# MarioCalvarro/circom_cvm

Measured on AMD Instinct MI355X. Metric: constraints simplified/sec (--O2) on 10M-constraint circuit; bit-exact .r1cs, higher is better.
Workload: dtype u64x4 (F_p, 256-bit Montgomery)

## Files before the change

circom_cvm_amd/abi.py:

```python
from __future__ import annotations

import ctypes as C

import numpy as np
import os

PKG = os.path.dirname(os.path.abspath(__file__))
LIB_PATH = os.environ.get("RS_LIB") or os.path.join(PKG, "librs_simplify.so")

U64_MAX = (1 << 64) - 1
PRIME_IDS = {"bn128": 0, "bls12381": 1, "goldilocks": 2, "grumpkin": 3, "pallas": 4,
             "vesta": 5, "secq256r1": 6, "bls12377": 7}
RS_PRIME_CUSTOM = 255
ERRORS = {0: "RS_OK", -1: "RS_E_INVALID", -2: "RS_E_OOM_DEVICE", -3: "RS_E_HIP",
          -4: "RS_E_RCCL", -5: "RS_E_INTERNAL", -6: "RS_E_NODEVICE"}


class RsLc(C.Structure):
    _fields_ = [("n_rows", C.c_uint64), ("nnz", C.c_uint64), ("ptr", C.POINTER(C.c_uint64)),
                ("col", C.POINTER(C.c_uint32)), ("val", C.POINTER(C.c_uint64))]


class RsInput(C.Structure):
    _fields_ = [("prime_id", C.c_uint32), ("prime", C.c_uint64 * 4), ("max_signal", C.c_uint64),
# ... 48 lines not shown
    if n == 0:
        return np.zeros(1, np.uint64), np.zeros(0, np.uint32), np.zeros(0, np.uint64)
    ext = int(lc.nnz)
    col = np.ctypeslib.as_array(lc.col, shape=(max(ext, 1),))
    val = np.ctypeslib.as_array(lc.val, shape=(max(ext, 1) * 4,))
    if layout is None:
        beg = np.ctypeslib.as_array(lc.ptr, shape=(n + 1,)).copy()
        nnz = int(beg[n])
        return beg, col[:nnz].copy(), val[:4 * nnz].copy()
    lp, jp, nj = layout
    lens = np.ctypeslib.as_array(lp, shape=(n,))
    jumps = np.ctypeslib.as_array(jp, shape=(nj,)) if nj else np.zeros(0, np.uint64)
    b = row_starts(lens, jumps)
    ln = (lens & ~np.uint32(ROW_JUMP)).astype(np.int64)
    if n and int((b + ln).max()) > ext:
        raise ValueError("row layout reaches past the block's entries")
    ptr = np.zeros(n + 1, np.uint64)
    np.cumsum(ln, out=ptr[1:])
    idx = np.repeat(b - ptr[:-1].astype(np.int64), ln) + np.arange(int(ptr[n]), dtype=np.int64)
    v4 = val[: 4 * ext].reshape(-1, 4)
    return ptr, col[idx].copy(), v4[idx].reshape(-1).copy()


class RsStats(C.Structure):
    _fields_ = [("total_ms", C.c_double), ("eq_ms", C.c_double), ("cluster_ms", C.c_double),
                ("elim_ms", C.c_double), ("subst_ms", C.c_double), ("final_ms", C.c_double),
                ("apply_kernel_ms", C.c_double), ("apply_kernel_launches", C.c_uint64),
                ("apply_bytes", C.c_uint64), ("elim_kernel_ms", C.c_double),
                ("elim_kernel_launches", C.c_uint64), ("elim_bytes", C.c_uint64),
                ("elim_big_ms", C.c_double), ("elim_small_ms", C.c_double), ("nl_ms", C.c_double),
                ("map_ms", C.c_double), ("rounds_ms", C.c_double),
                ("big_prep_ms", C.c_double), ("big_main_ms", C.c_double), ("big_finish_ms", C.c_double),
                ("big_main_bytes", C.c_uint64), ("big_finish_bytes", C.c_uint64), ("big_launches", C.c_uint64),
                ("rounds", C.c_uint64), ("n_clusters", C.c_uint64),
                ("n_substitutions", C.c_uint64), ("max_cluster", C.c_uint64),
                ("exchange_ms", C.c_double), ("exchange_bytes", C.c_uint64), ("world", C.c_uint64),
                ("head_main_ms", C.c_double), ("head_main_bytes", C.c_uint64), ("head_launches", C.c_uint64),
                ("tail_main_ms", C.c_double), ("tail_main_bytes", C.c_uint64), ("tail_launches", C.c_uint64),
                ("round_fill_ms", C.c_double), ("round_fill_bytes", C.c_uint64),
                ("round_fill_launches", C.c_uint64), ("alg_bytes", C.c_uint64), ("h2d_wait_ms", C.c_double),
                ("d2h_ms", C.c_double), ("host_total_ms", C.c_double), ("write_ms", C.c_double),
                ("tail_fin_ms", C.c_double), ("tail_fin_bytes", C.c_uint64), ("tail_fin_launches", C.c_uint64), ("head_fin_ms", C.c_double), ("head_fin_bytes", C.c_uint64), ("head_fin_launches", C.c_uint64), ("small_ms", C.c_double), ("small_bytes", C.c_uint64), ("small_launches", C.c_uint64), ("prep_ms", C.c_double), ("prep_launches", C.c_uint64), ("cluster_dev_ms", C.c_double), ("cluster_bytes", C.c_uint64), ("cluster_launches", C.c_uint64), ("giant_ms", C.c_double), ("giant_bytes", C.c_uint64), ("giant_launches", C.c_uint64), ("giant_merges", C.c_uint64),
                ("check_ms", C.c_double), ("check_bytes", C.c_uint64), ("check_launches", C.c_uint64),
                ("ragged_ms", C.c_double), ("ragged_bytes", C.c_uint64), ("ragged_launches", C.c_uint64),
                ("gather_ms", C.c_double), ("gather_bytes", C.c_uint64), ("gather_launches", C.c_uint64),
                ("cluster_host_ms", C.c_double),
                ("read_ms", C.c_double), ("read_upload_ms", C.c_double), ("read_kernel_ms", C.c_double),
                ("read_d2h_ms", C.c_double),
                ("sym_write_ms", C.c_double), ("sym_in_ms", C.c_double), ("sym_kernel_ms", C.c_double),
                ("sym_out_ms", C.c_double)]

    def as_dict(self):
        return {k: getattr(self, k) for k, _ in self._fields_}


class RsJsonStats(C.Structure):
    _fields_ = [("write_ms", C.c_double), ("in_ms", C.c_double), ("kernel_ms", C.c_double),
                ("out_ms", C.c_double), ("bytes", C.c_uint64)]

    def as_dict(self):
        return {k: getattr(self, k) for k, _ in self._fields_}


class RsWitness(C.Structure):
    _fields_ = [("prime_id", C.c_uint32), ("prime", C.c_uint64 * 4), ("n8", C.c_uint32), ("n", C.c_uint64),
                ("val", C.POINTER(C.c_uint64))]


WIT_INPUT, WIT_OUTPUT, WIT_LOG = 1, 2, 4
WIT_CLASSES = ("cons_eq", "eq", "linear", "nonlinear", "output", "log")


class RsWitnessReport(C.Structure):
    _fields_ = [("checked", C.c_uint64 * 6), ("failed", C.c_uint64 * 6), ("first_failed", C.c_uint64 * 6),
                ("in_ms", C.c_double), ("kernel_ms", C.c_double), ("total_ms", C.c_double)]

    def as_dict(self):
        d = {k: getattr(self, k) for k in ("in_ms", "kernel_ms", "total_ms")}
        for i, nm in enumerate(WIT_CLASSES):
            first = int(self.first_failed[i])
            d[nm] = {"checked": int(self.checked[i]), "failed": int(self.failed[i]),
                     "first_failed": None if first == U64_MAX else first}
        return d


class RsLiftReport(C.Structure):
    _fields_ = [("n_labels", C.c_uint64), ("n_wires", C.c_uint64), ("lifted", C.c_uint64), ("free_labels", C.c_uint64),
                ("shadowed", C.c_uint64), ("levels", C.c_uint64), ("entries", C.c_uint64),
                ("in_ms", C.c_double), ("kernel_ms", C.c_double), ("total_ms", C.c_double)]

    def as_dict(self):
        return {k: getattr(self, k) for k, _ in self._fields_}

    def counts(self):
        return tuple(int(getattr(self, k)) for k, t in self._fields_ if t is C.c_uint64)


class RsDag(C.Structure):
    _fields_ = [("prime_id", C.c_uint32), ("prime", C.c_uint64 * 4),
                ("n_pub_out", C.c_uint64), ("n_pub_in", C.c_uint64), ("n_priv_in", C.c_uint64),
                ("n_forbidden", C.c_uint64), ("forbidden", C.POINTER(C.c_uint32)),
                ("n_nodes", C.c_uint32), ("main_node", C.c_uint32),
                ("cons_off", C.POINTER(C.c_uint64)), ("a", RsLc), ("b", RsLc), ("c", RsLc),
                ("local_off", C.POINTER(C.c_uint64)), ("locals", C.POINTER(C.c_uint32)),
                ("custom_gate", C.POINTER(C.c_uint8)),
                ("edge_off", C.POINTER(C.c_uint64)), ("edge_to", C.POINTER(C.c_uint32)),
                ("edge_in", C.POINTER(C.c_uint64))]


SYMBOLS = [
    ("rs_last_error", C.c_char_p, []),
    ("rs_abi_version", C.c_int, []),
    ("rs_simplify", C.c_int, [C.POINTER(RsInput), C.POINTER(RsFlags), C.POINTER(C.POINTER(RsOutput))]),
    ("rs_output_free", None, [C.POINTER(RsOutput)]),
    ("rs_engine_create", C.c_int, [C.c_int, C.POINTER(C.c_void_p)]),
    ("rs_engine_load", C.c_int, [C.c_void_p, C.POINTER(RsInput)]),
    ("rs_engine_run", C.c_int, [C.c_void_p, C.POINTER(RsFlags)]),
    ("rs_engine_fetch", C.c_int, [C.c_void_p, C.POINTER(C.POINTER(RsOutput))]),
    ("rs_engine_stats", C.c_int, [C.c_void_p, C.POINTER(RsStats)]),
    ("rs_engine_destroy", None, [C.c_void_p]),
    ("rs_engine_write_r1cs", C.c_int, [C.c_void_p, C.c_char_p, C.c_char_p]),
    ("rs_engine_simplify", C.c_int, [C.c_void_p, C.POINTER(RsInput), C.POINTER(RsFlags),
                                     C.POINTER(C.POINTER(RsOutput))]),
    ("rs_host_alloc", C.c_void_p, [C.c_uint64]),
    ("rs_host_free", None, [C.c_void_p]),
    ("rs_comm_unique_id", C.c_int, [C.POINTER(C.c_uint8)]),
    ("rs_engine_join_rccl", C.c_int, [C.c_void_p, C.c_int, C.c_int, C.POINTER(C.c_uint8)]),
    ("rs_group_create", C.c_void_p, [C.c_int]),
    ("rs_engine_join_group", C.c_int, [C.c_void_p, C.c_void_p, C.c_int]),
    ("rs_engine_join_host", C.c_int, [C.c_void_p, C.c_int, C.c_int, C.c_char_p]),
    ("rs_group_destroy", None, [C.c_void_p]),
    ("rs_simplify_multi", C.c_int, [C.POINTER(RsInput), C.POINTER(RsFlags), C.c_int, C.POINTER(C.c_int),
                                    C.POINTER(C.POINTER(RsOutput))]),
    ("rs_engine_inject_fault", C.c_int, [C.c_void_p, C.c_int]),
    ("rs_read_r1cs_o0", C.c_int, [C.c_char_p, C.POINTER(C.POINTER(RsInput))]),
    ("rs_input_free", None, [C.POINTER(RsInput)]),
    ("rs_write_r1cs", C.c_int, [C.c_char_p, C.POINTER(RsInput), C.POINTER(RsOutput)]),
    ("rs_write_r1cs_gates", C.c_int, [C.c_char_p, C.POINTER(RsInput), C.POINTER(RsOutput), C.c_char_p]),
    ("rs_write_sym", C.c_int, [C.c_char_p, C.c_char_p, C.POINTER(RsOutput)]),
    ("rs_write_constraints_json", C.c_int, [C.c_char_p, C.POINTER(RsOutput)]),
    ("rs_write_substitution_json", C.c_int, [C.c_char_p, C.POINTER(RsOutput)]),
    ("rs_synth", C.c_int, [C.c_uint32, C.c_uint64, C.c_uint64, C.c_uint32, C.POINTER(C.POINTER(RsInput))]),
    ("rs_flatten_dag", C.c_int, [C.c_int, C.POINTER(RsDag), C.POINTER(C.POINTER(RsInput))]),
    ("rs_engine_flatten_dag", C.c_int, [C.c_void_p, C.POINTER(RsDag), C.POINTER(C.POINTER(RsInput))]),
    ("rs_engine_read_r1cs_o0", C.c_int, [C.c_void_p, C.c_char_p, C.POINTER(C.POINTER(RsInput))]),
    ("rs_read_r1cs_o0_device", C.c_int, [C.c_int, C.c_char_p, C.POINTER(C.POINTER(RsInput))]),
    ("rs_engine_write_sym", C.c_int, [C.c_void_p, C.c_char_p, C.c_char_p]),
    ("rs_write_sym_device", C.c_int, [C.c_int, C.c_char_p, C.c_char_p, C.POINTER(RsOutput)]),
    ("rs_engine_write_constraints_json", C.c_int, [C.c_void_p, C.c_char_p]),
    ("rs_engine_write_substitution_json", C.c_int, [C.c_void_p, C.c_char_p]),
    ("rs_write_constraints_json_device", C.c_int, [C.c_int, C.c_char_p, C.POINTER(RsOutput)]),
    ("rs_write_substitution_json_device", C.c_int, [C.c_int, C.c_char_p, C.POINTER(RsOutput)]),
    ("rs_engine_json_stats", C.c_int, [C.c_void_p, C.POINTER(RsJsonStats)]),
    ("rs_read_wtns", C.c_int, [C.c_char_p, C.POINTER(C.POINTER(RsWitness))]),
    ("rs_witness_free", None, [C.POINTER(RsWitness)]),
    ("rs_write_wtns", C.c_int, [C.c_char_p, C.POINTER(RsWitness), C.POINTER(RsOutput)]),
    ("rs_check_witness", C.c_int, [C.POINTER(RsInput), C.POINTER(RsOutput), C.POINTER(RsWitness), C.c_uint32,
                                   C.POINTER(RsWitnessReport)]),
    ("rs_engine_load_witness", C.c_int, [C.c_void_p, C.POINTER(RsWitness)]),
    ("rs_engine_load_wtns", C.c_int, [C.c_void_p, C.c_char_p]),
    ("rs_engine_check_witness", C.c_int, [C.c_void_p, C.POINTER(RsInput), C.c_uint32, C.POINTER(RsWitnessReport)]),
    ("rs_engine_write_wtns", C.c_int, [C.c_void_p, C.c_char_p]),
    ("rs_lift_witness", C.c_int, [C.POINTER(RsOutput), C.POINTER(RsWitness), C.POINTER(C.POINTER(RsWitness)),
                                  C.POINTER(RsLiftReport)]),
    ("rs_lift_witness_device", C.c_int, [C.c_int, C.POINTER(RsOutput), C.POINTER(RsWitness),
                                         C.POINTER(C.POINTER(RsWitness)), C.POINTER(RsLiftReport)]),
    ("rs_engine_lift_witness", C.c_int, [C.c_void_p, C.POINTER(RsLiftReport)]),
    ("rs_engine_fetch_witness", C.c_int, [C.c_void_p, C.POINTER(C.POINTER(RsWitness))]),
    ("rs_engine_write_wtns_resident", C.c_int, [C.c_void_p, C.c_char_p]),
]

_LIB = None


class RsError(RuntimeError):
    def __init__(self, code, msg):
        super().__init__(f"{ERRORS.get(code, code)}: {msg}")
        self.code = code


def lib():
    global _LIB
    if _LIB is None:
        if not os.path.exists(LIB_PATH):
            raise RuntimeError(f"{LIB_PATH} is missing: run `python -c 'import __graft_entry__ as g; g.build()'`")
        L = C.CDLL(LIB_PATH)
        for name, res, args in SYMBOLS:
            f = getattr(L, name)
            f.restype = res
            f.argtypes = args
        _LIB = L
    return _LIB


def check(rc: int):
    if rc != 0:
        raise RsError(rc, lib().rs_last_error().decode(errors="replace"))


def make_flags(level: str = "O2", rounds: int | None = None, old: bool = False, device: int = 0,
               log: bool = False) -> RsFlags:
    f = RsFlags()
    f.emit_substitution_log = 1 if log else 0
    if level == "O1" or rounds == 0:
        f.flag_s, f.no_rounds = 1, 0
    elif level == "O2":
# ... 78 lines not shown
        return p.contents

    def read_r1cs(self, path: str) -> RsInput:
        p = C.POINTER(RsInput)()
        check(lib().rs_engine_read_r1cs_o0(self._h, path.encode(), C.byref(p)))
        return p.contents

    def inject_fault(self, where: int = 1):
        check(lib().rs_engine_inject_fault(self._h, where))

    def write_r1cs(self, path: str, o0_r1cs: str | None = None) -> float:
        check(lib().rs_engine_write_r1cs(self._h, path.encode(), o0_r1cs.encode() if o0_r1cs else None))
        return self.stats().write_ms

    def write_sym(self, o0_sym: str, path: str) -> float:
        check(lib().rs_engine_write_sym(self._h, o0_sym.encode(), path.encode()))
        return self.stats().sym_write_ms

    def write_constraints_json(self, path: str) -> float:
        check(lib().rs_engine_write_constraints_json(self._h, path.encode()))
        return self.json_stats().write_ms

    def write_substitution_json(self, path: str) -> float:
        check(lib().rs_engine_write_substitution_json(self._h, path.encode()))
        return self.json_stats().write_ms

    def load_witness(self, w):
        check(lib().rs_engine_load_witness(self._h, C.byref(w.c if isinstance(w, Witness) else w)))

    def load_wtns(self, path: str):
        check(lib().rs_engine_load_wtns(self._h, path.encode()))

    def check_witness(self, what: int, inp: RsInput | None = None) -> RsWitnessReport:
        rep = RsWitnessReport()
        check(lib().rs_engine_check_witness(self._h, C.byref(inp) if inp is not None else None, what, C.byref(rep)))
        return rep

    def write_wtns(self, path: str):
        check(lib().rs_engine_write_wtns(self._h, path.encode()))

    def lift_witness(self) -> RsLiftReport:
        rep = RsLiftReport()
        check(lib().rs_engine_lift_witness(self._h, C.byref(rep)))
        return rep

    def fetch_witness(self) -> "Witness":
        p = C.POINTER(RsWitness)()
        check(lib().rs_engine_fetch_witness(self._h, C.byref(p)))
        return Witness(ptr=p)

    def write_wtns_resident(self, path: str):
        check(lib().rs_engine_write_wtns_resident(self._h, path.encode()))

    def json_stats(self) -> RsJsonStats:
        s = RsJsonStats()
        check(lib().rs_engine_json_stats(self._h, C.byref(s)))
        return s

    def close(self):
        if self._h:
            lib().rs_engine_destroy(self._h)
            self._h = C.c_void_p()

    def __del__(self):
        try:
            self.close()
        except Exception:
            pass


class Output:

    def __init__(self, ptr):
        self.ptr = ptr

    @property
    def c(self) -> RsOutput:
        s = self.ptr.contents
        s._owner = self
        return s

    @staticmethod
    def write_sym_device(o0_sym: str, path: str, out: RsOutput, device: int = 0):
        check(lib().rs_write_sym_device(device, o0_sym.encode(), path.encode(), C.byref(out)))

    @staticmethod
    def write_constraints_json_device(path: str, out: RsOutput, device: int = 0):
        check(lib().rs_write_constraints_json_device(device, path.encode(), C.byref(out)))

    @staticmethod
    def write_substitution_json_device(path: str, out: RsOutput, device: int = 0):
        check(lib().rs_write_substitution_json_device(device, path.encode(), C.byref(out)))

    def free(self):
        if self.ptr:
            lib().rs_output_free(self.ptr)
            self.ptr = None

    def __del__(self):
        try:
            self.free()
        except Exception:
            pass


def check_witness(w, what: int, inp: RsInput | None = None, out: RsOutput | None = None) -> RsWitnessReport:
# ... 169 lines not shown
```

circom_cvm_amd/csrc/engine.hip:

```cpp
#include <hip/hip_runtime.h>

#include <algorithm>
#include <atomic>
#include <chrono>
#include <condition_variable>
#include <cstdio>
#include <deque>
#include <mutex>
#include <map>
#include <memory>
#include <stdexcept>
#include <thread>
#include <string>
#include <unordered_map>
#include <unordered_set>
#include <functional>
#include <vector>

#include <cstring>
#include <fcntl.h>
#include <pthread.h>
#include <sched.h>
#include <sys/stat.h>
#include <unistd.h>
// ... 135 lines not shown
    if (n == ev.size()) {
      hipEvent_t e;
      HC(hipEventCreate(&e));
      ev.push_back(e);
    }
    HC(hipEventRecord(ev[n++], s));
  }
  template <class F>
  void run(hipStream_t s, uint64_t b, F &&f) {
    mark(s);
    f();
    mark(s);
    bytes += b;
  }
  void collect(double &ms, uint64_t &by, uint64_t &launches) {
    double t = 0;
    for (size_t i = 0; i + 1 < n; i += 2) {
      float m = 0;
      HC(hipEventSynchronize(ev[i + 1]));
      HC(hipEventElapsedTime(&m, ev[i], ev[i + 1]));
      t += m;
    }
    ms += t;
    by += bytes;
    launches += n ? 1 : 0;
    n = 0;
    bytes = 0;
  }
  void destroy() {
    for (hipEvent_t e : ev) (void)hipEventDestroy(e);
    ev.clear();
    n = 0;
  }
};

}
#include "comm.hpp"

using namespace rs;

enum Ev {
  kEvFill0, kEvFill1,
  kEvElim0, kEvElim1,
  kEvSmallFork,
  kEvTailPrep, kEvTailLoop,
  kEvTailEnd,
  kEvHead0, kEvHeadPrep, kEvHeadLoop, kEvHeadEnd,
  kEvHeadReady,
  kEvLane,
  kEvReplayFork, kEvReplayJoin,
  kEvNl0, kEvNl1,
  kEvCount
};
enum PinSlot {
  kPinPtr = 0,
  kPinCol = 3,
  kPinVal = 6,
  kPinL2w = 9,
  kPinWrite = 11,
  kPinLens = 13,
  kPinReplayMeta = 16,
  kPinReplayStage = 17,
  kPinRead = 18,
  kPinCluster = 19,
  kPinFlat = 20,
  kPinStage = 39,
  kPinCount = 40
};

struct rs_engine {
  uint64_t pool_want = 0;
  int device = 0;
  uint32_t n_cu = 256;
  hipStream_t st = nullptr;
  hipStream_t srd = nullptr;
  hipStream_t st2 = nullptr;
  hipEvent_t ev[kEvCount] = {};
  Arena A;
  Arena SA;
  bool loaded = false;
  bool have_result = false;
  int fault_at = 0;
  FieldP F;
  uint64_t prime[4];
  uint32_t prime_id = 0;
  uint64_t S = 0, n_pub_out = 0, n_pub_in = 0, n_priv_in = 0;
  std::vector<uint32_t> forbidden;
  struct Blk {
    uint64_t *ptr = nullptr;
    uint32_t *key = nullptr;
    Fe *val = nullptr;
    uint64_t n = 0, nnz = 0;
  } ce, eq, lin, na, nb, nc;
  uint64_t out_n_dev = 0;
  uint64_t out_nnz[3] = {0, 0, 0};
  uint64_t n_wires = 0, npiw = 0;
  rs_stats stats{};
  rs_json_stats jstats{};
  bool wit_on = false;
  uint64_t wit_n = 0;
  uint32_t wit_n8 = 0, wit_prime_id = 0;
  uint64_t wit_prime[4] = {0, 0, 0, 0};
  FieldP WF;
  std::unique_ptr<rs::Comm> comm;
  bool log_on = false;
  std::vector<uint32_t> log_from, log_key;
  std::vector<uint64_t> log_ptr, log_val;
  uint32_t *heap_k = nullptr;
  Fe *heap_v = nullptr;
  uint64_t heap_cap = 0;
  hipStream_t stc = nullptr;
  hipEvent_t ev_grp[4] = {};
  bool pending[4] = {false, false, false, false};
  int *h_vflag = nullptr;
  bool staged = false;
  const rs_input *hin = nullptr;
  unsigned long long *h_lvl = nullptr;
  hipEvent_t ev_lvl[4] = {};
  double h2d_wait_ms = 0;
  struct Pin {
    void *p = nullptr;
    size_t cap = 0;
  };
  Pin pin[kPinCount];
  rs_input flat_view{};
  rs_output view{};
  bool stream_out = false;
  bool snap_on = false;
  uint64_t snap_e[3] = {0, 0, 0};
  uint64_t out_ext[3] = {0, 0, 0};
  uint64_t nl_lo = 0, nl_hi = UINT64_MAX;
  uint64_t sh_cap[3] = {0, 0, 0};
  void *sh_ent = nullptr;
  bool sh_full = false;
  uint64_t sh_klo = 0, sh_khi = 0;
  uint64_t lc_snap_n = 0, lc_snap_base = 0;
  hipEvent_t ev_snap = nullptr, ev_snap0 = nullptr;
  uint64_t snap_cap[3] = {0, 0, 0};
  uint64_t snap_hint[3] = {0, 0, 0};
  void *snap_host[6] = {};
  struct SnapJob {
    void *dst;
    const void *src;
    size_t bytes;
    hipEvent_t ready;
  };
  hipEvent_t ev_snapq[6] = {};
  hipEvent_t ev_snaph[3] = {};
  double asm_t0_ms = 0, asm_end_ms = 0, snap_last_ms = 0;
  int snap_open = 0, asm_open = 0;
  hipEvent_t ev_fh[2] = {};
  hipEvent_t ev_nlc = nullptr;
  std::mutex snap_m;
  std::condition_variable snap_cv;
  std::deque<SnapJob> snap_q;
  bool snap_closed = true;
  std::thread snap_thread;
  cpu_set_t near_cpus;
  int near_n = 0;
  hipStream_t stx = nullptr;
  hipStream_t str = nullptr;
  hipStream_t ste = nullptr;
  hipStream_t stg = nullptr;
  hipEvent_t ev_gjoin = nullptr;
  hipEvent_t evt[2][5] = {};
  hipEvent_t evc[2] = {};
  hipEvent_t evgt[3] = {};
  hipEvent_t ev_sm[3] = {};
  hipEvent_t ev_chunk[8] = {};
  KGroup kg[3];
  int snap_rc = 0;
  bool csr_ready = false;
  bool csr_rows_ready = false;
  DRows fin_parts[3] = {}, fin_xq[2][3] = {};
  uint64_t out_njump[3] = {0, 0, 0};
  const uint32_t *fin_keep_ids = nullptr, *fin_x_ids[2] = {nullptr, nullptr};
  uint64_t fin_keep = 0, fin_xn[2] = {0, 0}, fin_gen = 0;
};

namespace rs {

enum UpPart { kUpAll = 0, kUpKeys = 1, kUpVals = 2 };

struct RowSplit {
  std::vector<uint64_t> lo, e;
};
static RowSplit split_rows(const rs_lc &src, int W, const char *name) {
  RowSplit sp;
  const uint64_t n = src.n_rows, nnz = n ? src.nnz : 0;
  sp.lo.assign(W + 1, 0);
  sp.e.assign(W + 1, 0);
  sp.lo[W] = n;
  sp.e[W] = nnz;
  if (n && (src.ptr[0] != 0 || src.ptr[n] != nnz))
    throw RsError(RS_E_INVALID, std::string(name) + " block: bad row pointers (ptr[0] != 0 or ptr[n_rows] != nnz)");
  for (int q = 1; q < W; ++q) {
    const uint64_t want = (unsigned __int128)nnz * q / W;
    uint64_t a = sp.lo[q - 1], b = n;
    while (a < b) {
      const uint64_t m = a + (b - a) / 2;
      if (src.ptr[m] < want) a = m + 1; else b = m;
    }
    sp.lo[q] = a;
    sp.e[q] = src.ptr[a];
// ... 190 lines not shown
static void snap_join(rs_engine *E);
static void *pin_get(rs_engine *E, int slot, size_t bytes);
static void ensure_csr(rs_engine *E);
static void load_abort(rs_engine *E) {
  if (E->stc) (void)hipStreamSynchronize(E->stc);
  snap_join(E);
  for (bool &pd : E->pending) pd = false;
  if (E->comm) E->comm->fail();
  for (hipStream_t q : {E->st, E->st2, E->ste, E->stg, E->stx, E->str})
    if (q) (void)hipStreamSynchronize(q);
}

static void rd(rs_engine *E, void *dst, const void *src, size_t bytes) {
  if (!bytes) return;
  HC(hipMemcpyAsync(dst, src, bytes, hipMemcpyDeviceToHost, E->srd));
  HC(hipStreamSynchronize(E->srd));
}
static void h2d(rs_engine *E, void *dst, const void *src, size_t bytes) {
  if (!bytes) return;
  HC(hipMemcpyAsync(dst, src, bytes, hipMemcpyHostToDevice, E->st));
  HC(hipStreamSynchronize(E->st));
}

template <class T, class Op>
static void excl_scan(Arena &A, const std::string &tag, hipStream_t s, const T *in, T *out, T zero, uint64_t n, Op op, bool size_only = false) {
  if (!n) return;
  size_t tb = 0;
  HC(rocprim::exclusive_scan(nullptr, tb, in, out, zero, (size_t)n, op, s));
  void *tmp = A.get<uint8_t>(tag, tb);
  if (!size_only) HC(rocprim::exclusive_scan(tmp, tb, in, out, zero, (size_t)n, op, s));
}

constexpr size_t kPinRb = 128;
static uint64_t excl_scan_u64(rs_engine *E, const uint64_t *in, uint64_t *out, uint64_t n, const char *tag,
                              double *waited = nullptr) {
  if (n == 0) return 0;
  excl_scan(E->A, std::string("scan.tmp.") + tag, E->st, in, out, (uint64_t)0, n, rocprim::plus<uint64_t>());
  uint64_t *h = (uint64_t *)pin_get(E, kPinRead, kPinRb) + 4;
  HC(hipMemcpyAsync(h, in + n - 1, 8, hipMemcpyDeviceToHost, E->st));
  HC(hipMemcpyAsync(h + 1, out + n - 1, 8, hipMemcpyDeviceToHost, E->st));
  const double t0 = waited ? now_ms() : 0.0;
  HC(hipStreamSynchronize(E->st));
  if (waited) *waited += now_ms() - t0;
  return h[0] + h[1];
}

struct U3 {
  uint64_t a, b, c;
};
struct U3Plus {
  __host__ __device__ U3 operator()(const U3 &x, const U3 &y) const { return U3{x.a + y.a, x.b + y.b, x.c + y.c}; }
};
static U3 excl_scan_u3(rs_engine *E, const U3 *in, U3 *out, uint64_t n, const char *tag, const uint64_t *x_in = nullptr,
                       const uint64_t *x_out = nullptr, uint64_t *x_sum = nullptr) {
  if (n == 0 && !x_sum) return U3{0, 0, 0};
  uint64_t *h = (uint64_t *)pin_get(E, kPinRead, kPinRb) + 8;
  if (n) {
    excl_scan(E->A, std::string("scan3.tmp.") + tag, E->st, in, out, U3{0, 0, 0}, n, U3Plus());
    HC(hipMemcpyAsync(h, in + n - 1, sizeof(U3), hipMemcpyDeviceToHost, E->st));
    HC(hipMemcpyAsync(h + 3, out + n - 1, sizeof(U3), hipMemcpyDeviceToHost, E->st));
  }
  if (x_sum) {
    HC(hipMemcpyAsync(h + 6, x_in, 8, hipMemcpyDeviceToHost, E->st));
    HC(hipMemcpyAsync(h + 7, x_out, 8, hipMemcpyDeviceToHost, E->st));
  }
  HC(hipStreamSynchronize(E->st));
  if (x_sum) *x_sum = h[6] + h[7];
  return n ? U3{h[0] + h[3], h[1] + h[4], h[2] + h[5]} : U3{0, 0, 0};
}

#include "stage_io.hpp"
#include "flatten.hpp"
#include "r1cs_read.hpp"
#include "sym_write.hpp"
#include "json_write.hpp"
#include "witness.hpp"
#include "lift.hpp"
#include "output.hpp"
__global__ void k_pack3(const uint64_t *a, const uint64_t *b, const uint64_t *c, uint64_t n, U3 *out) {
  for (uint64_t i = gtid(); i < n; i += gstride()) out[i] = U3{a[i], b[i], c[i]};
}
__global__ void k_set_offsets_u3(const U3 *scan, uint64_t ba, uint64_t bb, uint64_t bc, uint64_t n, uint64_t *oa, uint64_t *ob,
                                 uint64_t *oc, const U3 *cap, const uint32_t *ids) {
  for (uint64_t i = gtid(); i < n; i += gstride()) {
    if (cap && cap[i].a == 0) continue;
    const uint64_t r = ids ? ids[i] : i;
    oa[r] = ba + scan[i].a;
    ob[r] = bb + scan[i].b;
    oc[r] = bc + scan[i].c;
  }
}

__global__ void k_mark_u8(const uint32_t *ids, uint64_t n, uint8_t *flag) {
  for (uint64_t i = gtid(); i < n; i += gstride()) flag[ids[i]] = 1;
}

__global__ void k_append_marks(const uint32_t *usig, const uint64_t *uoff, const uint32_t *ulen, uint64_t nU,
                               const uint32_t *pk, uint8_t *nlmap) {
  for (uint64_t i = gtid(); i < nU; i += gstride()) {
    if (!nlmap[usig[i]]) continue;
    for (uint32_t t = 0; t < ulen[i]; ++t) nlmap[pk[uoff[i] + t]] = 1;
  }
}

template <class K, class V>
static void sort_pairs(rs_engine *E, const K *kin, K *kout, const V *vin, V *vout, uint64_t n, int end_bit,
                       const char *tag, hipStream_t s = nullptr) {
  if (!n) return;
  if (!s) s = E->st;
  size_t tb = 0;
  HC(rocprim::radix_sort_pairs(nullptr, tb, kin, kout, vin, vout, (size_t)n, 0, end_bit, s));
  void *tmp = E->A.get<uint8_t>(std::string("sort.tmp.") + tag, tb);
  HC(rocprim::radix_sort_pairs(tmp, tb, kin, kout, vin, vout, (size_t)n, 0, end_bit, s));
}
static void dev_scan_u64(rs_engine *E, const uint64_t *in, uint64_t *out, uint64_t n, hipStream_t s, const char *tag) {
  excl_scan(E->A, std::string("scan.tmp.") + tag, s, in, out, (uint64_t)0, n, rocprim::plus<uint64_t>());
}
static void dev_scan_u3(rs_engine *E, const U3 *in, U3 *out, uint64_t n, hipStream_t s, const char *tag) {
  excl_scan(E->A, std::string("scan3.tmp.") + tag, s, in, out, U3{0, 0, 0}, n, U3Plus());
// ... 779 lines not shown
  hipLaunchKernelGGL(k_gi_union, dim3(gb), dim3(256), 0, s, a, G, c);
  hipLaunchKernelGGL(k_gi_rowkey, dim3(gb), dim3(256), 0, s, a, G, c);
  HC(hipGetLastError());
  sort_pairs(E, (const uint64_t *)G.rkey, G.rkey2, (const uint32_t *)G.rval, G.rval2, n, 64, "gi", s);
  hipLaunchKernelGGL(k_gi_segment, dim3(1), dim3(1024), 0, s, a, G);
  HC(hipGetLastError());
  sort_pairs(E, (const uint64_t *)G.ckey, G.ckey2, (const uint32_t *)G.cidx, G.cidx2, n, 64, "gi", s);
  if (g_prof_env) {
    HC(hipMemsetAsync(G.sec, 0, 256, s));
    HC(hipStreamSynchronize(s));
  }
  const double tl0 = g_prof_env ? now_ms() : 0.0;
  hipLaunchKernelGGL(k_gi_loop, dim3((unsigned)std::min<uint64_t>(n, 512)), dim3(kGhThreads), 0, s, a, G, c);
  HC(hipGetLastError());
  if (g_prof_env) {
    HC(hipStreamSynchronize(s));
    const double tl1 = now_ms();
    uint32_t nc = 0;
    HC(hipMemcpy(&nc, G.scal, 4, hipMemcpyDeviceToHost));
    std::vector<uint32_t> sz(nc), mg(nc);
    std::vector<uint64_t> ck(nc);
    if (nc) {
      HC(hipMemcpy(sz.data(), G.c_size, 4 * nc, hipMemcpyDeviceToHost));
      HC(hipMemcpy(mg.data(), G.c_merges, 4 * nc, hipMemcpyDeviceToHost));
      HC(hipMemcpy(ck.data(), G.c_clk, 8 * nc, hipMemcpyDeviceToHost));
    }
    std::vector<uint32_t> ord(nc);
    for (uint32_t i = 0; i < nc; ++i) ord[i] = i;
    std::sort(ord.begin(), ord.end(), [&](uint32_t x, uint32_t y) { return ck[x] > ck[y]; });
    uint64_t tm = 0, tc = 0;
    for (uint32_t i = 0; i < nc; ++i) { tm += mg[i]; tc += ck[i]; }
    fprintf(stderr, "[rs-prof] giant %llu rows: %u components, %llu merges, loop %.1f ms (sum of component times %.1f ms)\n",
            (unsigned long long)n, nc, (unsigned long long)tm, tl1 - tl0, tc / 1e5);
    for (uint32_t i = 0; i < nc && i < 8; ++i)
      fprintf(stderr, "[rs-prof]   component rows %u merges %u: %.1f ms (%.2f us/merge)\n", sz[ord[i]], mg[ord[i]], ck[ord[i]] / 1e5,
              mg[ord[i]] ? ck[ord[i]] / 1e2 / mg[ord[i]] : 0.0);
    unsigned long long sec[32];
    HC(hipMemcpy(sec, G.sec, 256, hipMemcpyDeviceToHost));
    const double nm = (double)std::max<uint64_t>(tm, 1);
    fprintf(stderr, "[rs-prof]   loop clocks per merge, slot side: decide %.0f | to B' %.0f | combine+B %.0f | rebuild %.0f | row start %.0f | "
            "row end %.0f | serial %.0f\n", sec[0] / nm, sec[1] / nm, sec[2] / nm, sec[3] / nm, sec[4] / nm, sec[5] / nm, sec[6] / nm);
    fprintf(stderr, "[rs-prof]   loop clocks per merge, RHS side: decide %.0f | loads %.0f | find %.0f | product %.0f | insert %.0f | B' %.0f | "
            "B %.0f\n", sec[16] / nm, sec[24] / nm, sec[25] / nm, sec[26] / nm, sec[27] / nm, sec[17] / nm, sec[18] / nm);
  }
  dev_scan_u32(E, G.c_nsub, G.c_dsub, n, s, "gi");
  hipLaunchKernelGGL(k_gi_gather, dim3(gb), dim3(256), 0, s, a, G, c);
  HC(hipGetLastError());
  dev_scan_u32(E, G.lmark, G.lscan, n, s, "gi");
  hipLaunchKernelGGL(k_gi_scatter, dim3(gb), dim3(256), 0, s, a, G, c);
  hipLaunchKernelGGL(k_gi_fin, dim3(1), dim3(64), 0, s, a, G, c);
  HC(hipGetLastError());
}

using HeadOverlap = std::function<void(const uint32_t *head_ids, uint64_t n_head, const ElimArgs &a)>;

static void run_linear_simplification(rs_engine *E, const DRows &view, int old_heur, ElimOut &eo, Pool &P,
                                      int *d_err, uint8_t *d_forb, int32_t *sub_of, uint8_t *deleted,
                                      const HeadOverlap *overlap = nullptr,
                                      const std::function<void()> *before_elim = nullptr,
                                      const uint8_t *need = nullptr) {
  double t0 = now_ms();
  if (E->fault_at == 1) {
    E->fault_at = 0;
    throw RsError(RS_E_INTERNAL, "injected fault (rs_engine_inject_fault)");
  }
  DevClusters D = gpu_clusters(E, view, old_heur, d_forb, eo);
  if (before_elim) (*before_elim)();
  double t1 = now_ms();
  E->stats.cluster_ms += t1 - t0;
  const uint64_t n_slots = D.n_slots, tot_nnz = D.tot_nnz;
  uint64_t n_big = D.n_big, n_small = D.n_small;
  uint32_t *d_perm = D.perm, *d_big = D.big, *d_small = D.small, *d_cid = D.cid;
  uint64_t *d_cl = D.cl_off;
  Comm *CM = E->comm.get();
  const int W = CM ? CM->world : 1, RK = CM ? CM->rank : 0;
  uint8_t *d_owner = nullptr;
  const uint64_t n_rep = std::min<uint64_t>(n_big, kHeadLimit);
  if (W > 1 && eo.n_clusters) {
    d_owner = E->A.get<uint8_t>("sh.owner", eo.n_clusters);
    const uint64_t n_tb = n_big - n_rep;
    if (n_rep) launch(E->st, k_fill_u8_ids, n_rep, (const uint32_t *)d_big, n_rep, (uint8_t)W, d_owner);
    if (n_tb) launch(E->st, k_shard_owner, n_tb, (const uint32_t *)(d_big + n_rep), n_tb, W, d_owner);
    if (n_small) launch(E->st, k_shard_owner, n_small, (const uint32_t *)d_small, n_small, W, d_owner);
    const uint64_t nb = snake_count(n_tb, W, RK), ns = snake_count(n_small, W, RK);
    uint32_t *bb = E->A.get<uint32_t>("sh.big", n_rep + nb), *ss = E->A.get<uint32_t>("sh.small", ns);
    if (n_rep) HC(hipMemcpyAsync(bb, d_big, 4 * n_rep, hipMemcpyDeviceToDevice, E->st));
    if (nb) launch(E->st, k_shard_pick, nb, (const uint32_t *)(d_big + n_rep), nb, W, RK, bb + n_rep);
    if (ns) launch(E->st, k_shard_pick, ns, (const uint32_t *)d_small, ns, W, RK, ss);
    d_big = bb;
    d_small = ss;
    n_big = n_rep + nb;
    n_small = ns;
  }
  uint64_t want = std::max<uint64_t>(std::max<uint64_t>(1 << 20, 8 * (tot_nnz + n_slots)), E->pool_want);
  {
    uint64_t giant_rows_sum = 0;
    for (uint64_t i = 0; i < std::min<uint64_t>(n_big, kHeadLimit) && i < D.top_keys.size(); ++i) {
      const uint64_t r = (0xffffffffull - (D.top_keys[i] >> 32)) & 0x7fffffffull;
      if (r >= kGiantRows && !D.order_free.count((uint32_t)(D.top_keys[i] & 0xffffffffull))) giant_rows_sum += r;
    }
    if (!env_flag("RS_GI_NOPOOL")) want = std::max<uint64_t>(want, 192 * giant_rows_sum);
  }
  for (int attempt = 0; attempt < 8; ++attempt) {
    P = get_pool(E, want);
    Pool G{};
    bool exchanged = false;
    HC(hipMemsetAsync(P.top, 0, 8, E->st));
// ... 105 lines not shown
          const dim3 g2(kWideX, g);
          const uint32_t *ids = d_big;
          hipLaunchKernelGGL(k_wide_alloc, dim3(g), dim3(256), 0, E->st2, a, ids, n_head);
          hipLaunchKernelGGL(k_wide_count, g2, dim3(256), 0, E->st2, a, ids, n_head);
          hipLaunchKernelGGL(k_wide_conv, g2, dim3(256), 0, E->st2, a, ids, n_head);
          hipLaunchKernelGGL(k_wide_uniq, g2, dim3(256), 0, E->st2, a, ids, n_head);
          hipLaunchKernelGGL(k_wide_remove, g2, dim3(256), 0, E->st2, a, ids, n_head);
          hipLaunchKernelGGL(k_wide_clear, g2, dim3(256), 0, E->st2, a, ids, n_head);
          HC(hipGetLastError());
        }
        hipLaunchKernelGGL(k_big_prep, dim3(g), dim3(256), 0, E->st2, a, (const uint32_t *)d_big, n_head);
        HC(hipGetLastError());
        HC(hipEventRecord(E->ev[kEvHeadPrep], E->st2));
        HC(hipEventRecord(E->ev[kEvHeadReady], E->st2));
        if (!giants.empty()) {
          HC(hipStreamWaitEvent(E->stg, E->ev[kEvHeadReady], 0));
          HC(hipMemsetAsync(GA.scal + 5, 0, 4, E->stg));
          HC(hipEventRecord(E->evgt[0], E->stg));
          ElimArgs ag = a;
          ag.bytes_main = a.bytes + 7;
          for (uint64_t i : giants) {
            GiantArgs G = GA;
            G.n = (0xffffffffull - (D.top_keys[i] >> 32)) & 0x7fffffffull;
            giant_launch(E, ag, G, D.top_keys[i] & 0xffffffffull, i);
          }
          HC(hipEventRecord(E->evgt[1], E->stg));
          HC(hipEventRecord(E->ev_gjoin, E->stg));
        }
        hipLaunchKernelGGL(k_big_spec<12>, dim3(g), dim3(768), 0, E->st2, aspec, (const uint32_t *)d_big, n_head);
        HC(hipGetLastError());
        HC(hipEventRecord(E->ev[kEvHeadLoop], E->st2));
        if (!giants.empty()) HC(hipStreamWaitEvent(E->st2, E->ev_gjoin, 0));
        HC(hipEventRecord(E->evgt[2], E->st2));
        hipLaunchKernelGGL(k_batch_inv_tree, dim3(g), dim3(256), 0, E->st2, a, (const uint32_t *)d_big, n_head);
        HC(hipGetLastError());
        hipLaunchKernelGGL(k_normalize, dim3(16, g), dim3(256), 0, E->st2, ah, (const uint32_t *)d_big, n_head);
        HC(hipGetLastError());
        hipLaunchKernelGGL(k_big_finish<8>, dim3(g), dim3(512), 0, E->st2, ah, (const uint32_t *)d_big, n_head, 0u);
        HC(hipGetLastError());
      }
      if (n_head) HC(hipStreamWaitEvent(E->st, E->ev[kEvHeadReady], 0));
      HC(hipEventRecord(E->ev[kEvSmallFork], E->st));
      HC(hipStreamWaitEvent(E->ste, E->ev[kEvSmallFork], 0));
      HC(hipEventRecord(E->ev_sm[0], E->ste));
      if (n_small) {
        uint64_t blocks = (n_small + 63) / 64;
        hipLaunchKernelGGL(k_eliminate, dim3((unsigned)std::min<uint64_t>(blocks, 1u << 20)), dim3(64), 0, E->ste, a,
                           (const uint32_t *)d_small, (uint64_t)n_small);
        HC(hipGetLastError());
      }
      HC(hipEventRecord(E->ev_sm[1], E->ste));
      HC(hipEventRecord(E->ev[kEvLane], E->st));
      n_tgroups = 0;
      if (n_tail) {
        static const uint64_t split = env_u64("RS_TAIL_SPLIT", kTailSplit, 1, UINT64_MAX / 2);
        const uint64_t n_t1 = n_tail > split + split / 4 ? split : n_tail, n_t2 = n_tail - n_t1;
        n_tgroups = n_t2 ? 2 : 1;
        auto tail_group = [&](hipStream_t s, ElimArgs g, const uint32_t *ids, uint64_t n, const char *cls_name, int grp) {
          const bool timed = grp == 0;
          hipEvent_t *ev = E->evt[grp];
          const unsigned gb = (unsigned)std::min<uint64_t>(n, 2048), gm = (unsigned)std::min<uint64_t>(n, 8192);
          HC(hipEventRecord(ev[0], s));
          hipLaunchKernelGGL(k_big_prep, dim3(gb), dim3(256), 0, s, g, ids, n);
          HC(hipGetLastError());
          HC(hipMemsetAsync(g.skip, 0, n, s));
          hipLaunchKernelGGL(k_p3_fast, dim3(gb), dim3(256), 0, s, g, ids, n);
          HC(hipGetLastError());
          if (timed) HC(hipEventRecord(E->ev[kEvTailPrep], s));
          HC(hipEventRecord(ev[1], s));
          hipLaunchKernelGGL(k_big_main<256>, dim3(gm), dim3(64), 0, s, g, ids, n);
          HC(hipGetLastError());
          if (timed) HC(hipEventRecord(E->ev[kEvTailLoop], s));
          HC(hipEventRecord(ev[2], s));
          {
            uint8_t *cls = E->A.get<uint8_t>(cls_name, eo.n_clusters);
            HC(hipMemsetAsync(cls, 0, eo.n_clusters, s));
            launch(s, k_mark_u8, n, ids, n, cls);
            launch(s, k_batch_inv_flat, (n_slots + 63) / 64, g, (const uint32_t *)d_cid, (const uint8_t *)cls, n_slots);
          }
          HC(hipEventRecord(ev[3], s));
          hipLaunchKernelGGL(k_big_finish<4>, dim3(gb), dim3(256), 0, s, g, ids, n, kFinWaveBelow);
          HC(hipGetLastError());
          HC(hipEventRecord(ev[4], s));
        };
        uint8_t *skip = E->A.get<uint8_t>("el.skip", n_tail);
        at.skip = skip;
        tail_group(E->st, at, d_big + n_head, n_t1, "el.cls", 0);
        if (n_t2) {
          ElimArgs a2 = at;
          a2.big_touch_off += n_t1;
          a2.big_touch_n += n_t1;
          a2.big_alive += n_t1;
          a2.skip = skip + n_t1;
          if (a2.prof) a2.prof += kProfWords * n_t1;
          tail_group(E->ste, a2, d_big + n_head + n_t1, n_t2, "el.cls2", 1);
        }
      }
      HC(hipEventRecord(E->ev_sm[2], E->ste));
      if (n_head) {
        hl.ah = ah;
        hl.ids = d_big;
        hl.s = E->st2;
        hl.cur = ah.cf_items;
        hl.nxt = cf_next;
        hl.n_slots = n_slots;
        hl.h = E->h_lvl;
        hl.ev = E->ev_lvl;
        if (overlap) hl.run(std::min(kHeadGpuLevels, kHeadLevels), false);
      }
      HC(hipEventRecord(E->ev[kEvTailEnd], E->st));
      HC(hipStreamWaitEvent(E->st, E->ev_sm[2], 0));
      if (D.join_pending) {
        HC(hipStreamWaitEvent(E->st, E->ev[kEvReplayJoin], 0));
        D.join_pending = false;
      }
      auto finish_head = [&] {
        hl.run(kHeadGpuLevels, false);
        if (!hl.done) {
          hipLaunchKernelGGL(k_compose_rest<8>, dim3((unsigned)n_head), dim3(512), 0, E->st2, ah, (const uint32_t *)d_big,
                             (const uint64_t *)hl.cur, (const unsigned long long *)(ah.cf_n + hl.level % 3), n_head);
          HC(hipGetLastError());
        }
        hipLaunchKernelGGL(k_big_emit<8>, dim3((unsigned)n_head), dim3(512), 0, E->st2, ah, (const uint32_t *)d_big, n_head);
        HC(hipGetLastError());
        HC(hipEventRecord(E->ev[kEvHeadEnd], E->st2));
        if (g_prof_env) fprintf(stderr, "[rs-prof] head composition: %u level launches\n", hl.levels);
      };
      if (n_head) finish_head();
      if (W > 1) {
        int e0 = 0;
        HC(hipMemcpyAsync(&e0, d_err, 4, hipMemcpyDeviceToHost, E->st));
        HC(hipStreamSynchronize(E->st));
        exchanged = CM->max_u64((uint32_t)e0, E->st) == 0;
        if (exchanged) shard_exchange(E, a, D, d_owner, P, need, G);
      }
      if (n_head && overlap && (W == 1 || exchanged)) {
        ElimArgs ao = a;
        if (W > 1) {
          ao.pk = G.pk;
          ao.pv = G.pv;
        }
        (*overlap)(d_big, n_head, ao);
      }
      if (n_head) HC(hipStreamWaitEvent(E->st, E->ev[kEvHeadEnd], 0));
      HC(hipEventRecord(E->ev[kEvElim1], E->st));
    }
    unsigned long long *d_sums = E->A.get<unsigned long long>("el.sums", 2);
    auto sum_counts = [&](unsigned long long *h) {
      HC(hipMemsetAsync(d_sums, 0, 16, E->st));
      if (eo.n_clusters) launch_capped(E->st, k_sum_counts, eo.n_clusters, 256, (const uint32_t *)a.n_sub, (const uint32_t *)a.n_left,
                                       eo.n_clusters, d_sums);
      HC(hipMemcpyAsync(h, d_sums, 16, hipMemcpyDeviceToHost, E->st));
    };
    unsigned long long sums[2] = {0, 0};
    int err = 0;
    sum_counts(sums);
    HC(hipMemcpyAsync(&err, d_err, 4, hipMemcpyDeviceToHost, E->st));
    HC(hipStreamSynchronize(E->st));
    if (W > 1) {
      const uint64_t mine = (uint32_t)err;
      err = 0;
      for (uint64_t x : CM->gather_u64(mine, E->st)) err |= (int)x;
    }
    if ((err & 8) && !(err & kGiErrBounds)) {
      size_t fr_ = 0, tot_ = 0;
      (void)hipMemGetInfo(&fr_, &tot_);
      if (g_prof_env) {
        unsigned long long used = 0;
        HC(hipMemcpy(&used, P.top, 8, hipMemcpyDeviceToHost));
        fprintf(stderr, "[rs-debug] pool exhausted: cap %llu entries, top %llu, attempt %d\n",
                (unsigned long long)want, used, attempt);
      }
      want = std::min<uint64_t>(want * 2, (uint64_t)(fr_ * 0.8) / 36 + want / 2);
      continue;
    }
    if (err) throw RsError(RS_E_INTERNAL, "elimination invariant violated (code " + std::to_string(err) + ")");
    E->pool_want = std::max(E->pool_want, want);
    if (g_prof_env) {
      unsigned long long used = 0;
      HC(hipMemcpy(&used, P.top, 8, hipMemcpyDeviceToHost));
      fprintf(stderr, "[rs-prof] pool: %llu of %llu entries (%.2f per cluster entry)\n", used, (unsigned long long)want,
                (double)used / (double)std::max<uint64_t>(1, tot_nnz + n_slots));
    }
    if (W > 1 && eo.n_clusters) {
      unsigned long long top = 0;
      HC(hipMemcpyAsync(&top, P.top, 8, hipMemcpyDeviceToHost, E->st));
      HC(hipStreamSynchronize(E->st));
      const uint64_t base = G.cap;
      E->A.grow_keep<uint32_t>("pool.gk", base + top + 1, base, E->st, E->st);
      E->A.grow_keep<Fe>("pool.gv", base + top + 1, base, E->st, E->st);
      uint32_t *gk = E->A.get<uint32_t>("pool.gk", 1);
      Fe *gv = E->A.get<Fe>("pool.gv", 1);
      if (top) {
        HC(hipMemcpyAsync(gk + base, P.pk, 4 * top, hipMemcpyDeviceToDevice, E->st));
        HC(hipMemcpyAsync(gv + base, P.pv, 32 * top, hipMemcpyDeviceToDevice, E->st));
// ... 634 lines not shown
    HC(hipGetDeviceProperties(&prop, device));
    if (std::string(prop.gcnArchName).find("gfx950") == std::string::npos) {
      set_error(std::string("device is ") + prop.gcnArchName + ", this build targets gfx950 only");
      return RS_E_NODEVICE;
    }
    std::unique_ptr<rs_engine> E(new rs_engine());
    E->device = device;
    CPU_ZERO(&E->near_cpus);
    E->near_n = near_gpu_cpus(device, &E->near_cpus);
    if (g_prof_env && E->near_n) fprintf(stderr, "[rs-prof] engine calls run on the GPU's %d local CPUs\n", E->near_n);
    E->n_cu = (uint32_t)prop.multiProcessorCount;
    const bool pooled = env_flag("RS_POOLED_STREAMS"), all_masked = env_flag("RS_CUMASK_STREAMS");
    std::vector<uint32_t> cu_mask((E->n_cu + 31) / 32, 0u);
    for (uint32_t c = 0; c < E->n_cu; ++c) cu_mask[c / 32] |= 1u << (c % 32);
    auto mk_stream = [&](hipStream_t *sp, bool dedicated) {
      if (pooled || !dedicated || hipExtStreamCreateWithCUMask(sp, (uint32_t)cu_mask.size(), cu_mask.data()) != hipSuccess)
        HC(hipStreamCreateWithFlags(sp, hipStreamNonBlocking));
    };
    mk_stream(&E->st, all_masked);
    HC(hipStreamCreateWithFlags(&E->srd, hipStreamNonBlocking));
    {
      int lo = 0, hi = 0;
      if (hipDeviceGetStreamPriorityRange(&lo, &hi) != hipSuccess ||
          hipStreamCreateWithPriority(&E->st2, hipStreamNonBlocking, hi) != hipSuccess)
        HC(hipStreamCreateWithFlags(&E->st2, hipStreamNonBlocking));
    }
    mk_stream(&E->stc, true);
    mk_stream(&E->stx, all_masked);
    mk_stream(&E->str, all_masked);
    {
      int lo = 0, hi = 0;
      if (env_flag("RS_STE_DEFAULT") || hipDeviceGetStreamPriorityRange(&lo, &hi) != hipSuccess ||
          hipStreamCreateWithPriority(&E->ste, hipStreamNonBlocking, lo) != hipSuccess)
        HC(hipStreamCreateWithFlags(&E->ste, hipStreamNonBlocking));
      if (g_prof_env) fprintf(stderr, "[rs-prof] stream priorities: least %d greatest %d\n", lo, hi);
    }
    mk_stream(&E->stg, all_masked);
    HC(hipEventCreateWithFlags(&E->ev_gjoin, hipEventDisableTiming));
    for (auto &g : E->evt)
      for (auto &ev : g) HC(hipEventCreate(&ev));
    for (auto &ev : E->evc) HC(hipEventCreate(&ev));
    for (auto &ev : E->evgt) HC(hipEventCreate(&ev));
    for (auto &ev : E->ev_sm) HC(hipEventCreate(&ev));
    for (auto &ev : E->ev) HC(hipEventCreate(&ev));
    for (auto &ev : E->ev_grp) HC(hipEventCreateWithFlags(&ev, hipEventDisableTiming));
    HC(hipHostMalloc((void **)&E->h_vflag, 10 * sizeof(int), hipHostMallocDefault));
    memset(E->h_vflag, 0, 10 * sizeof(int));
    HC(hipHostMalloc((void **)&E->h_lvl, 8 * sizeof(unsigned long long), hipHostMallocDefault));
    for (auto &ev : E->ev_lvl) HC(hipEventCreateWithFlags(&ev, hipEventDisableTiming));
    HC(hipEventCreateWithFlags(&E->ev_snap, hipEventDisableTiming));
    HC(hipEventCreateWithFlags(&E->ev_snap0, hipEventDisableTiming));
    for (auto &ev : E->ev_chunk) HC(hipEventCreateWithFlags(&ev, hipEventDisableTiming));
    for (auto &ev : E->ev_snapq) HC(hipEventCreateWithFlags(&ev, hipEventDisableTiming));
    for (auto &ev : E->ev_snaph) HC(hipEventCreateWithFlags(&ev, hipEventDisableTiming));
    for (auto &ev : E->ev_fh) HC(hipEventCreate(&ev));
    HC(hipEventCreateWithFlags(&E->ev_nlc, hipEventDisableTiming));
    *eng = E.release();
    return RS_OK;
  } catch (const RsError &e) {
    set_error(e.what());
    return e.code;
  } catch (const std::exception &e) {
    set_error(e.what());
    return RS_E_INTERNAL;
  }
}

void rs_engine_destroy(rs_engine *E) {
  if (!E) return;
  (void)hipSetDevice(E->device);
  if (E->st) (void)hipStreamSynchronize(E->st);
  if (E->st2) (void)hipStreamSynchronize(E->st2);
  if (E->stc) (void)hipStreamSynchronize(E->stc);
  if (E->ste) (void)hipStreamSynchronize(E->ste);
  if (E->stg) (void)hipStreamSynchronize(E->stg);
  snap_join(E);
  E->comm.reset();
  for (auto &pb : E->pin)
    if (pb.p) (void)hipHostFree(pb.p);
  if (E->h_vflag) (void)hipHostFree(E->h_vflag);
  if (E->h_lvl) (void)hipHostFree(E->h_lvl);
  for (auto &ev : E->ev_lvl)
    if (ev) (void)hipEventDestroy(ev);
  for (auto &ev : E->ev_grp)
    if (ev) (void)hipEventDestroy(ev);
  for (auto &g : E->kg) g.destroy();
  if (E->stc) (void)hipStreamDestroy(E->stc);
  if (E->stx) (void)hipStreamDestroy(E->stx);
  if (E->str) (void)hipStreamDestroy(E->str);
  if (E->ste) (void)hipStreamDestroy(E->ste);
  if (E->stg) (void)hipStreamDestroy(E->stg);
  if (E->srd) (void)hipStreamDestroy(E->srd);
  if (E->ev_gjoin) (void)hipEventDestroy(E->ev_gjoin);
  for (auto &g : E->evt)
    for (auto &ev : g)
      if (ev) (void)hipEventDestroy(ev);
  for (auto &ev : E->evc)
    if (ev) (void)hipEventDestroy(ev);
  for (auto &ev : E->evgt)
    if (ev) (void)hipEventDestroy(ev);
  for (auto &ev : E->ev_sm)
    if (ev) (void)hipEventDestroy(ev);
  if (E->ev_snap) (void)hipEventDestroy(E->ev_snap);
  if (E->ev_snap0) (void)hipEventDestroy(E->ev_snap0);
  for (auto &ev : E->ev_chunk)
    if (ev) (void)hipEventDestroy(ev);
  for (auto &ev : E->ev_snapq)
    if (ev) (void)hipEventDestroy(ev);
  if (E->heap_k) (void)hipFree(E->heap_k);
  if (E->heap_v) (void)hipFree(E->heap_v);
  if (E->st) (void)hipStreamDestroy(E->st);
  if (E->st2) (void)hipStreamDestroy(E->st2);
  for (auto &ev : E->ev)
    if (ev) (void)hipEventDestroy(ev);
  delete E;
}

int rs_engine_load(rs_engine *E, const rs_input *in) {
  CpuNear cpu_near_(E);
  CallScope cs(E);
  try {
    HC(hipSetDevice(E->device));
    load_enqueue(E, in, false);
    load_wait_all(E);
    cs.ok = true;
    return RS_OK;
  } catch (const RsError &e) {
    load_abort(E);
    E->loaded = false;
    set_error(e.what());
    return e.code;
  } catch (const std::exception &e) {
    load_abort(E);
    E->loaded = false;
    set_error(e.what());
    return RS_E_INTERNAL;
  }
}

int rs_engine_run(rs_engine *E, const rs_flags *fl) {
  CpuNear cpu_near_(E);
  CallScope cs(E);
  try {
    if (!E->loaded) { set_error("engine has no input"); return RS_E_INVALID; }
    HC(hipSetDevice(E->device));
    engine_run(E, fl);
    cs.ok = true;
    return RS_OK;
  } catch (const RsError &e) {
    set_error(e.what());
    return e.code;
  } catch (const std::exception &e) {
    set_error(e.what());
    return RS_E_INTERNAL;
  }
}

int rs_engine_stats(rs_engine *E, rs_stats *s) {
  *s = E->stats;
  return RS_OK;
}
// ... 401 lines not shown
    const char *nm[3] = {"out.a", "out.b", "out.c"};
    JsonSrc s;
    s.n = E->out_n_dev;
    s.nparts = 3;
    for (int q = 0; q < 3; ++q) {
      s.ptr[q] = E->A.get<uint64_t>(std::string(nm[q]) + ".ptr", 1);
      s.col[q] = E->A.get<uint32_t>(std::string(nm[q]) + ".col", 1);
      s.val[q] = E->A.get<uint64_t>(std::string(nm[q]) + ".val", 1);
      s.nnz[q] = E->out_nnz[q];
    }
    s.l2w = E->A.get<int32_t>("fin.l2w", 1);
    s.n_labels = E->S;
    write_json_device(E, s, path, t0, t0);
    return RS_OK;
  });
}

int rs_engine_write_substitution_json(rs_engine *E, const char *path) {
  if (!E || !path) { set_error("rs_engine_write_substitution_json: null argument"); return RS_E_INVALID; }
  return engine_call(E, true, [&]() -> int {
    if (!E->have_result) throw RsError(RS_E_INVALID, "no result");
    if (env_flag("RS_WRITER_HOST")) return json_via_host(E, path, true);
    const double t0 = now_ms();
    JsonSrc s;
    s.nparts = 1;
    s.n = E->log_on ? E->log_from.size() : 0;
    double t_in = t0;
    if (s.n) {
      const uint64_t n = s.n, nnz = E->log_key.size();
      if (E->log_ptr.size() != n + 1 || E->log_ptr[n] != nnz || E->log_val.size() != 4 * nnz)
        throw RsError(RS_E_INTERNAL, "the substitution log's arrays disagree");
      Arena &A = E->SA;
      uint32_t *from = A.get<uint32_t>("json.log.from", n), *key = A.get<uint32_t>("json.log.key", nnz);
      uint64_t *ptr = A.get<uint64_t>("json.log.ptr", n + 1), *val = A.get<uint64_t>("json.log.val", 4 * nnz);
      const uint64_t all = 4 * n + 8 * (n + 1) + 36 * nnz;
      StageIn up(E, (all + 4095) & ~4095ull);
      up.send(from, E->log_from.data(), 4 * n);
      up.send(ptr, E->log_ptr.data(), 8 * (n + 1));
      up.send(key, E->log_key.data(), 4 * nnz);
      up.send(val, E->log_val.data(), 32 * nnz);
      HC(hipStreamSynchronize(E->stc));
      t_in = now_ms();
      s.from = from;
      s.ptr[0] = ptr;
      s.col[0] = key;
      s.val[0] = val;
      s.nnz[0] = nnz;
    }
    write_json_device(E, s, path, t0, t_in);
    return RS_OK;
  });
}

int rs_engine_json_stats(rs_engine *E, rs_json_stats *st) {
  if (!E || !st) { set_error("rs_engine_json_stats: null argument"); return RS_E_INVALID; }
  *st = E->jstats;
  return RS_OK;
}

int rs_write_constraints_json_device(int device, const char *path, const rs_output *out) {
  if (!path || !out || (out->n_labels && !out->label_to_wire)) {
    set_error("rs_write_constraints_json_device: null argument");
    return RS_E_INVALID;
  }
  return one_shot(device, [&](rs_engine *E) {
    const double t0 = now_ms();
    const rs_lc *L[3] = {&out->a, &out->b, &out->c};
    const uint32_t *len[3] = {out->a_len, out->b_len, out->c_len};
    const char *nm[3] = {"json.in.a", "json.in.b", "json.in.c"};
    JsonHostPart hp[3];
    JsonSrc s;
    s.n = out->n_constraints;
    s.nparts = 3;
    for (int q = 0; q < 3; ++q) {
      json_host_part(out, q, *L[q], s.n, len[q], hp[q]);
      json_upload_part(E, hp[q], s.n, nm[q], q, s);
    }
    int32_t *l2w = E->SA.get<int32_t>("json.in.l2w", out->n_labels);
    if (out->n_labels) HC(hipMemcpyAsync(l2w, out->label_to_wire, 4 * out->n_labels, hipMemcpyHostToDevice, E->st));
    HC(hipStreamSynchronize(E->st));
    s.l2w = l2w;
    s.n_labels = out->n_labels;
    write_json_device(E, s, path, t0, now_ms());
  });
}

int rs_write_substitution_json_device(int device, const char *path, const rs_output *out) {
  if (!path || !out || (out->n_log && (!out->log_from || !out->log_to.ptr))) {
    set_error("rs_write_substitution_json_device: null argument");
    return RS_E_INVALID;
  }
  return one_shot(device, [&](rs_engine *E) {
    const double t0 = now_ms();
    JsonHostPart hp;
    JsonSrc s;
    s.n = out->n_log;
    s.nparts = 1;
    json_host_part(nullptr, 0, out->log_to, s.n, nullptr, hp);
    json_upload_part(E, hp, s.n, "json.in.log", 0, s);
    if (s.n) {
      uint32_t *from = E->SA.get<uint32_t>("json.in.from", s.n);
      HC(hipMemcpyAsync(from, out->log_from, 4 * s.n, hipMemcpyHostToDevice, E->st));
      s.from = from;
    }
    HC(hipStreamSynchronize(E->st));
    write_json_device(E, s, path, t0, now_ms());
// ... 261 lines not shown
```

circom_cvm_amd/csrc/frames_wave.hpp:

```cpp
#pragma once

namespace rs {

#ifndef FW_T
#define FW_T 640
#endif
#ifndef FW_E
#define FW_E 320
#endif
#ifndef FW_OCC
#define FW_OCC 2
#endif
constexpr uint32_t kFwT = FW_T;
constexpr uint32_t kFwE = FW_E;
constexpr uint32_t kFwG = 192;
constexpr uint32_t kFwPT = kFwT / 64;
constexpr uint32_t kFwPE = kFwE / 64;
constexpr uint32_t kFwWaves = 4;
constexpr uint32_t kFwRunsRank = 8;
#ifndef FW_KB
#define FW_KB 2
#endif

struct FrameWaveArgs {
  FrameArgs fr;
  DRows in[3], out[3];
  const uint64_t *cap[3];
  int cap_by_row;
  const uint32_t *ids;
  uint64_t n;
  uint64_t x0;
  const uint64_t *late;
  uint32_t *big;
  unsigned *n_big;
  int round;
  uint8_t *touched;
  uint32_t *turn_list;
  unsigned *n_turn;
  int *err;
  unsigned long long *bytes;
  unsigned long long *clk;
};

#ifdef RS_FWCLK
#define FW_CLK(i)                                                                      \
  do {                                                                                 \
    const unsigned long long now_ = clock64();                                         \
    clk_acc[i] += now_ - clk_last;                                                     \
    clk_last = now_;                                                                   \
  } while (0)
#else
#define FW_CLK(i) do { } while (0)
#endif
#ifdef RS_FWCLK
#define FW_WAIT() asm volatile("s_waitcnt vmcnt(0) lgkmcnt(0)" ::: "memory")
#else
#define FW_WAIT() do { } while (0)
#endif

struct FwLds {
  uint32_t tkey[kFwT];
  uint32_t tsrc[kFwT];
  uint16_t perm[kFwT];
  uint64_t nzm[kFwPT + 1];
  uint32_t nzp[kFwPT + 1];
  uint16_t e_t0[kFwE + 1];
  uint32_t e_key[kFwE];
  uint8_t e_kind[kFwE];
  uint8_t e_grp[kFwE];
  uint16_t e_pos[kFwE];
  uint64_t e_aux[kFwE];
  uint16_t g_e0[kFwG + 1];
  uint16_t g_t0[kFwG + 1];
  uint64_t g_in[kFwG];
  uint64_t g_out[kFwG];
  uint32_t g_k0[kFwG];
  uint64_t fx_off[3][64];
  uint32_t fx_row[64];
  uint32_t fx_cc[64];
  uint32_t fx_len[3][64];
  uint8_t fx_other[64];
};

__device__ __forceinline__ uint32_t fw_scan(uint32_t x, uint32_t lane) {
// ... 556 lines not shown
    const bool clear = len[0] == 0 || len[1] == 0;
    if (!clear && (ca || cb)) {
      other = ca ? 1 : 0;
    } else {
      if (clear) len[0] = len[1] = 0;
#pragma unroll
      for (int p = 0; p < 3; ++p) A.out[p].len[r] = len[p];
      bytes += 36ull * (len[0] + len[1] + len[2]);
      if (A.round && clear) {
        const unsigned pos = atomicAdd(A.n_turn, 1u);
        A.turn_list[pos] = (uint32_t)r;
      }
    }
  }
  const uint64_t fm = __ballot(other >= 0);
  if (fm) {
    const uint32_t nfix = (uint32_t)__popcll(fm);
    const uint32_t tw = other >= 0 ? len[2] + len[other] : 0u, tsum = __shfl(fw_scan(tw, lane), 63);
    if (fx_n + nfix > 64 || fx_terms + tsum > kFwT) {
      fw_fix(A, L, lane, fx_n, bytes FW_CLK_ARGS);
      fx_n = 0;
      fx_terms = 0;
    }
    if (other >= 0) {
      const uint32_t q = fx_n + (uint32_t)__popcll(fm & fw_below(lane));
      L.fx_row[q] = (uint32_t)r;
      L.fx_cc[q] = cc;
      L.fx_other[q] = (uint8_t)other;
#pragma unroll
      for (int p = 0; p < 3; ++p) {
        L.fx_off[p][q] = ooff[p];
        L.fx_len[p][q] = len[p];
      }
    }
    fx_n += nfix;
    fx_terms += tsum;
  }
  (void)x_of_row;
  wave_sync();
  FW_CLK(6);
}

template <int kRound>
__global__ __launch_bounds__(256, FW_OCC) void k_frames_wave(FrameWaveArgs A) {
  __shared__ FwLds lds[kFwWaves];
  const uint32_t lane = threadIdx.x & 63, wv = threadIdx.x >> 6;
  FwLds &L = lds[wv];
  unsigned long long bytes = 0;
#ifdef RS_FWCLK
  unsigned long long clk_last = clock64(), clk_k0 = clk_last, clk_acc[20] = {};
#endif
  const uint64_t nw = (uint64_t)gridDim.x * kFwWaves;
  uint32_t fx_n = 0, fx_terms = 0;
  for (uint64_t base = A.x0 + ((uint64_t)blockIdx.x * kFwWaves + wv) * 64; base < A.n; base += nw * 64) {
    const uint64_t x = base + lane;
    bool act = x < A.n;
    uint64_t r = 0, ioff[3] = {0, 0, 0}, ooff[3] = {0, 0, 0};
    uint32_t ln[3] = {0, 0, 0}, wt = 0, cc = 0;
    if (act) {
      r = A.ids ? A.ids[x] : x;
      const bool late = A.late && A.late[r];
      const uint64_t ci = A.cap_by_row ? r : x;
      const uint64_t ca = A.cap[0][ci], cb = A.cap[1][ci], cc2 = A.cap[2][ci];
#pragma unroll
      for (int p = 0; p < 3; ++p) {
        ln[p] = A.in[p].len[r];
        ioff[p] = A.in[p].off[r];
        ooff[p] = A.out[p].off[r];
      }
      if (late) {
        act = false;
      } else {
        if (A.round) A.touched[r] = 1;
        const uint64_t mx = ca > cb ? ca : cb, c3 = (cc2 - mx) / 2;
        cc = (uint32_t)c3;
        const uint64_t t = (ca - 1 - ln[0]) + (cb - 1 - ln[1]) + (c3 - 1 - ln[2]);
        if (t > kFwT || (uint64_t)ln[0] + ln[1] + ln[2] > kFwE) {
          const unsigned pos = atomicAdd(A.n_big, 1u);
          A.big[pos] = (uint32_t)(A.cap_by_row ? r : x);
          act = false;
        } else {
          wt = (uint32_t)t;
        }
      }
    }
    if (!act) ln[0] = ln[1] = ln[2] = 0;
    FW_CLK(7);
    const uint32_t P = fw_scan(wt, lane), Q = fw_scan(ln[0] + ln[1] + ln[2], lane);
    uint32_t s = 0;
    while (s < 64) {
      const uint32_t bp = s ? __shfl(P, s - 1) : 0, bq = s ? __shfl(Q, s - 1) : 0;
      const uint64_t bad = __ballot(lane >= s && (P - bp > kFwT || Q - bq > kFwE));
      const uint32_t e = bad ? (uint32_t)__builtin_ctzll(bad) : 64u;
      const bool inb = act && lane >= s && lane < e;
#ifdef RS_FWCLK
      if (__ballot(inb)) fw_batch(A, L, lane, inb, r, ln, ioff, ooff, cc, x, fx_n, fx_terms, bytes, clk_acc);
      clk_last = clock64();
      clk_acc[8] += 1;
#else
      if (__ballot(inb)) fw_batch(A, L, lane, inb, r, ln, ioff, ooff, cc, x, fx_n, fx_terms, bytes);
#endif
      s = e;
    }
  }
  if (fx_n) {
#ifdef RS_FWCLK
    unsigned long long clk_last2 = clock64();
// ... 16 lines not shown
```

circom_cvm_amd/csrc/kernels.hpp:

```cpp
#pragma once
#include <hip/hip_runtime.h>

#include "field.hpp"

namespace rs {

#define RS_NONE 0xffffffffu
constexpr uint64_t kProfWords = 24;

struct DRows {
  uint64_t *off;
  uint32_t *len;
  uint32_t *key;
  Fe *val;
  uint64_t n;
};

__device__ __forceinline__ uint64_t gtid() { return (uint64_t)blockIdx.x * blockDim.x + threadIdx.x; }
__device__ __forceinline__ uint64_t gstride() { return (uint64_t)gridDim.x * blockDim.x; }
__device__ __forceinline__ void wave_atomic_add(unsigned long long *p, unsigned long long x) {
#pragma unroll
  for (int d = 32; d >= 1; d >>= 1) x += __shfl_xor(x, d);
  if ((threadIdx.x & 63) == 0 && x) atomicAdd(p, x);
}
// ... 2921 lines not shown
    }
  if (any) n = d_sort_combine(F, tk, tv, n);
  if (A.ce_has) {
    any = false;
    for (uint32_t i = 0; i < n; ++i)
      if (A.ce_has[tk[i]]) { tv[i] = fmul(F, tv[i], A.ce_val[tk[i]]); tk[i] = 0; any = true; }
    if (any) n = d_sort_combine(F, tk, tv, n);
  }
  {
    uint32_t w;
    if (d_frame3_merge<8>(A, k, v, base, n, w)) return w;
  }
  uint32_t rb = cap - n;
  if (rb != base)
    for (uint32_t i = n; i-- > 0;) { k[rb + i] = tk[i]; v[rb + i] = tv[i]; }
  uint32_t w = 0;
  any = false;
  for (uint32_t i = 0; i < n; ++i) {
    uint32_t kk = k[rb + i];
    Fe vv = v[rb + i];
    int32_t s = A.sub_of[kk];
    if (s >= 0) {
      any = true;
      const uint32_t *rk = A.pk + A.h_off[s];
      const Fe *rv = A.pv + A.h_off[s];
      uint32_t rl = A.h_len[s];
      for (uint32_t j = 0; j < rl; ++j) { k[w] = rk[j]; v[w] = fmul(F, vv, rv[j]); ++w; }
    } else {
      k[w] = kk;
      v[w] = vv;
      ++w;
    }
  }
  if (any) w = d_sort_combine(F, k, v, w);
  return d_drop_zeros(k, v, w);
}

struct NLArgs {
  FrameArgs fr;
  DRows a, b, c;
  DRows oa, ob, oc;
  uint64_t *cap_a, *cap_b, *cap_c;
  unsigned long long *bytes;
  const uint32_t *ids;
  uint64_t n;
  int phase;
  const uint8_t *hmark;
  uint64_t *late;
  const uint32_t *xlist;
  const unsigned *n_xlist;
};

__global__ void k_mark_head_keys(DRows rows, const uint32_t *perm, const uint64_t *cl_off, const uint32_t *ids,
                                 uint8_t *hmark) {
  const uint32_t c = ids[blockIdx.y];
  const uint64_t b = cl_off[c], e = cl_off[c + 1];
  for (uint64_t i = b + blockIdx.x * blockDim.x + threadIdx.x; i < e; i += (uint64_t)gridDim.x * blockDim.x) {
    const uint32_t r = perm[i];
    const uint64_t o = rows.off[r];
    for (uint32_t j = 0; j < rows.len[r]; ++j) {
      const uint32_t k = rows.key[o + j];
      if (k) hmark[k] = 1;
    }
  }
}

__device__ inline bool d_touches_head(const FrameArgs &F, const uint8_t *hmark, const DRows &R, uint64_t r) {
  const uint64_t o = R.off[r];
  for (uint32_t i = 0; i < R.len[r]; ++i) {
    const uint32_t k = R.key[o + i];
    const int32_t t = F.eq_rep ? F.eq_rep[k] : -1;
    const uint32_t k1 = t >= 0 ? (uint32_t)t : k;
    if (F.ce_has && F.ce_has[k1]) continue;
    if (hmark[k1]) return true;
  }
  return false;
}

__global__ void k_nl_count(NLArgs A) {
  for (uint64_t x = gtid(); x < A.n; x += gstride()) {
    const uint64_t r = A.ids ? A.ids[x] : x;
    if (A.phase == 1) {
      const bool lt = d_touches_head(A.fr, A.hmark, A.a, r) || d_touches_head(A.fr, A.hmark, A.b, r) ||
                      d_touches_head(A.fr, A.hmark, A.c, r);
      A.late[r] = lt;
      if (lt) {
        A.cap_a[x] = A.cap_b[x] = A.cap_c[x] = 0;
        continue;
      }
    }
    uint64_t ca = 1 + A.a.len[r], cb = 1 + A.b.len[r], cc = 1 + A.c.len[r];
    for (uint32_t i = 0; i < A.a.len[r]; ++i) ca += d_frame_weight(A.fr, A.a.key[A.a.off[r] + i]);
    for (uint32_t i = 0; i < A.b.len[r]; ++i) cb += d_frame_weight(A.fr, A.b.key[A.b.off[r] + i]);
    for (uint32_t i = 0; i < A.c.len[r]; ++i) cc += d_frame_weight(A.fr, A.c.key[A.c.off[r] + i]);
    A.cap_a[x] = ca;
    A.cap_b[x] = cb;
    A.cap_c[x] = 2 * cc + (ca > cb ? ca : cb);
  }
}

__global__ void k_nl_fill(NLArgs A) {
  unsigned long long bytes = 0;
  const uint64_t nx = A.xlist ? *A.n_xlist : A.n;
  for (uint64_t xi = gtid(); xi < nx; xi += gstride()) {
    const uint64_t x = A.xlist ? A.xlist[xi] : xi;
    const uint64_t r = A.ids ? A.ids[x] : x;
    if (A.phase == 1 && A.late[r]) continue;
    uint64_t oa = A.oa.off[r], ob = A.ob.off[r], oc = A.oc.off[r];
    uint32_t capa = (uint32_t)A.cap_a[x], capb = (uint32_t)A.cap_b[x];
    uint32_t capc = (uint32_t)A.cap_c[x];
    uint32_t mx = capa > capb ? capa : capb;
    uint32_t cc = (capc - mx) / 2;
    uint32_t na = d_apply_frames(A.fr, A.a.key + A.a.off[r], A.a.val + A.a.off[r], A.a.len[r], A.oa.key + oa, A.oa.val + oa, capa);
    uint32_t nb = d_apply_frames(A.fr, A.b.key + A.b.off[r], A.b.val + A.b.off[r], A.b.len[r], A.ob.key + ob, A.ob.val + ob, capb);
    uint32_t nc = d_apply_frames(A.fr, A.c.key + A.c.off[r], A.c.val + A.c.off[r], A.c.len[r], A.oc.key + oc, A.oc.val + oc, cc);
    d_fix(A.fr.F, A.oa.key + oa, A.oa.val + oa, na, A.ob.key + ob, A.ob.val + ob, nb, A.oc.key + oc, A.oc.val + oc,
// ... 339 lines not shown
```

circom_cvm_amd/csrc/output.hpp:

```cpp
#pragma once

__device__ __forceinline__ uint64_t u3_sel(const U3 &x, int q) { return q == 0 ? x.a : (q == 1 ? x.b : x.c); }

struct ViewCopy {
  uint64_t *off[3];
  uint32_t *len[3];
};
__device__ __forceinline__ void view_copy(const ViewCopy &v, const DRows &a, const DRows &b, const DRows &c, uint64_t i,
                                          uint32_t la, uint32_t lb, uint32_t lc) {
  v.off[0][i] = a.off[i];
  v.off[1][i] = b.off[i];
  v.off[2][i] = c.off[i];
  v.len[0][i] = la;
  v.len[1][i] = lb;
  v.len[2][i] = lc;
}

__global__ void k_snap_flags(DRows a, DRows b, DRows c, const uint64_t *late, uint64_t n, uint64_t lo, uint64_t hi, uint8_t *early,
                             U3 *elen, ViewCopy vc) {
  for (uint64_t i = gtid(); i < n; i += gstride()) {
    const bool done = (!late || !late[i]) && i >= lo && i < hi;
    const uint32_t la = done ? a.len[i] : 0, lb = done ? b.len[i] : 0, lc = done ? c.len[i] : 0;
    const bool ok = (la | lb) != 0;
    early[i] = ok ? 1 : 0;
    elen[i] = ok ? U3{la, lb, lc} : U3{0, 0, 0};
    if (ok) view_copy(vc, a, b, c, i, la, lb, lc);
  }
}

__global__ void k_snap_lens2_l(DRows a, DRows b, DRows c, const uint32_t *ids, uint64_t n, U3 *elen, ViewCopy vc) {
  for (uint64_t i = gtid(); i < n; i += gstride()) {
    const uint32_t r = ids[i];
    const uint32_t la = a.len[r], lb = b.len[r], lc = c.len[r];
    const bool ok = (la | lb) != 0;
    elen[i] = ok ? U3{la, lb, lc} : U3{0, 0, 0};
    if (ok) view_copy(vc, a, b, c, r, la, lb, lc);
  }
}
__global__ void k_snap_mark2_l(const uint32_t *ids, const U3 *elen, const U3 *eoff2, U3 base, uint64_t n, uint8_t *early, U3 *eoff) {
  for (uint64_t i = gtid(); i < n; i += gstride()) {
    if ((elen[i].a | elen[i].b) == 0) continue;
    const uint32_t r = ids[i];
    early[r] = 1;
    eoff[r] = U3{base.a + eoff2[i].a, base.b + eoff2[i].b, base.c + eoff2[i].c};
  }
}

__global__ void k_snap_lens_rng(DRows a, DRows b, DRows c, const uint64_t *late, uint64_t lo, uint64_t hi, uint64_t n, U3 *elen,
                                ViewCopy vc) {
  for (uint64_t i = gtid(); i < n; i += gstride()) {
    const bool ok = i >= lo && i < hi && !(late && late[i]) && (a.len[i] | b.len[i]) != 0;
    elen[i] = ok ? U3{a.len[i], b.len[i], c.len[i]} : U3{0, 0, 0};
    if (ok) view_copy(vc, a, b, c, i, a.len[i], b.len[i], c.len[i]);
  }
}
__global__ void k_snap_mark_sel(const U3 *elen, const U3 *eoff2, U3 base, uint64_t n, uint8_t *early, U3 *eoff) {
  for (uint64_t i = gtid(); i < n; i += gstride()) {
    if ((elen[i].a | elen[i].b) == 0) continue;
    early[i] = 1;
    eoff[i] = U3{base.a + eoff2[i].a, base.b + eoff2[i].b, base.c + eoff2[i].c};
  }
}

__global__ void k_snap_gather(FieldP F, DRows R, const uint8_t *early, const U3 *eoff, int q, uint64_t n, uint32_t *col,
                              uint64_t *val, const uint64_t *only, uint64_t lo) {
  for (uint64_t r = lo + gtid(); r < n; r += gstride()) {
    if (!early[r] || (only && !only[r])) continue;
    const uint64_t o = u3_sel(eoff[r], q), s = R.off[r];
    const uint32_t len = R.len[r];
    for (uint32_t t = 0; t < len; ++t) {
      col[o + t] = R.key[s + t];
      const Fe c = ffrom_mont(F, R.val[s + t]);
      val[4 * (o + t) + 0] = c.l[0];
      val[4 * (o + t) + 1] = c.l[1];
      val[4 * (o + t) + 2] = c.l[2];
      val[4 * (o + t) + 3] = c.l[3];
    }
  }
}

__global__ void k_snap_gather_l(FieldP F, DRows R, const uint32_t *ids, const U3 *elen, const U3 *eoff, int q, uint64_t n,
                                uint32_t *col, uint64_t *val) {
  for (uint64_t i = gtid(); i < n; i += gstride()) {
    if ((elen[i].a | elen[i].b) == 0) continue;
    const uint32_t r = ids[i];
    const uint64_t o = u3_sel(eoff[r], q), s = R.off[r];
    const uint32_t len = R.len[r];
    for (uint32_t t = 0; t < len; ++t) {
      col[o + t] = R.key[s + t];
      const Fe c = ffrom_mont(F, R.val[s + t]);
      val[4 * (o + t) + 0] = c.l[0];
      val[4 * (o + t) + 1] = c.l[1];
      val[4 * (o + t) + 2] = c.l[2];
      val[4 * (o + t) + 3] = c.l[3];
    }
  }
}

__global__ void k_snap_lens_round(DRows a, DRows b, DRows c, const uint8_t *touched, const int32_t *turn, const uint32_t *nl_of,
                                  const uint8_t *early, uint64_t n, U3 *elen, ViewCopy vc) {
  for (uint64_t r = gtid(); r < n; r += gstride()) {
    const bool ok = (touched[r] || !early[nl_of[r]]) && turn[r] < 0 && (a.len[r] | b.len[r]) != 0;
    elen[r] = ok ? U3{a.len[r], b.len[r], c.len[r]} : U3{0, 0, 0};
    if (ok) view_copy(vc, a, b, c, r, a.len[r], b.len[r], c.len[r]);
  }
}
__global__ void k_snap_mark_round(const uint32_t *nl_of, const U3 *elen, const U3 *eoff3, U3 base, uint64_t n, uint8_t *early,
                                  U3 *eoff, uint8_t *dirty) {
  for (uint64_t r = gtid(); r < n; r += gstride()) {
    if ((elen[r].a | elen[r].b) == 0) continue;
    const uint32_t i = nl_of[r];
    early[i] = 1;
    eoff[i] = U3{base.a + eoff3[r].a, base.b + eoff3[r].b, base.c + eoff3[r].c};
    dirty[r] = 0;
  }
}
__global__ void k_snap_gather_st(FieldP F, DRows R, const U3 *elen, const U3 *eoff3, uint64_t base, int q, uint64_t n,
                                 uint32_t *col, uint64_t *val) {
  for (uint64_t r = gtid(); r < n; r += gstride()) {
// ... 307 lines not shown
```

circom_cvm_amd/csrc/run.hpp:

```cpp
#pragma once

static std::string part_name(const char *pre, int q, const char *suf) { return std::string(pre) + "abc"[q] + suf; }

constexpr uint64_t kUncMin = 1024, kUncDiv = 16;

struct Run {
  rs_engine *const E;
  const rs_flags *const fl;
  Arena &A;
  const hipStream_t st;
  const uint64_t S;
  KGroup &kg1;
  const bool apply_linear;
  uint64_t no_rounds;
  double T0 = 0, Tf = 0;
  int *d_err = nullptr;
  uint8_t *d_forb = nullptr, *d_deleted = nullptr;
  int32_t *sub_of = nullptr, *eq_rep = nullptr;
  uint8_t *ce_has = nullptr;
  Fe *ce_val = nullptr;
  LcHeap lc;
  DRows ce{}, lin{};
  bool keys_first = false;
  uint8_t *lin_fixed = nullptr;
  const uint64_t n_nl;
  DRows nl_in[3] = {};
  bool nl_staged = false;
  DRows stor[3] = {};
  uint64_t heap_top = 0;
  uint32_t *heap_k = nullptr;
  Fe *heap_v = nullptr;
  unsigned long long *d_bytes = nullptr;
  int *d_fw_err = nullptr;
  FrameArgs fr;
  uint64_t *cap[3] = {};
  U3 *cap3 = nullptr, *sc3 = nullptr;
  uint64_t *nl_late = nullptr, *nl_lpos = nullptr;
  uint8_t *hmark = nullptr;
  uint32_t *nl_lids = nullptr;
  uint64_t n_late = 0;
  bool nl_split = false;
  bool fh_split = false;
  uint8_t *so_early = nullptr;
  U3 *so_eoff = nullptr;
  uint8_t *so_dirty = nullptr;
  ElimOut eo;
  Pool P;
  uint64_t n_st = 0, n_wl = 0;
  uint32_t *st_ids = nullptr, *wl_ids = nullptr;
  DRows sv[3] = {};
  uint8_t *nlmap = nullptr;
  DRows lv{};
  bool apply_round = false;
  DRows m0[3] = {};
  MapLists ML;
  uint8_t *qflag = nullptr;
  int32_t *rank_of = nullptr, *r_sub_of = nullptr;
  ElimOut er;
  Marks MK;
  uint64_t nU = 0;
  uint32_t *d_us = nullptr, *d_ulen = nullptr;
  uint64_t *d_uoff = nullptr;
  std::vector<uint32_t> usig;
  std::vector<std::pair<uint64_t, uint32_t>> turned;

  Run(rs_engine *e, const rs_flags *f)
      : E(e), fl(f), A(e->A), st(e->st), S(e->S), kg1(e->kg[1]), apply_linear(!f->flag_s), no_rounds(f->no_rounds), n_nl(e->na.n) {}

  void init() {
    E->stats = rs_stats{};
    E->stats.world = E->comm ? (uint64_t)E->comm->world : 1;
    for (int g = 1; g < 3; ++g) {
      E->kg[g].n = 0;
      E->kg[g].bytes = 0;
    }
    if (E->A.defer || !E->A.graveyard.empty()) {
      for (hipStream_t q : {E->st, E->st2, E->stc, E->ste, E->stg})
        if (q) (void)hipStreamSynchronize(q);
      E->A.defer = false;
      E->A.flush();
    }
    T0 = now_ms();
    d_err = A.get<int>("err", 1);
    HC(hipMemsetAsync(d_err, 0, 4, st));

    d_forb = A.get<uint8_t>("forb", S);
    d_deleted = A.get<uint8_t>("deleted", S);
    HC(hipMemsetAsync(d_forb, 0, S, st));
    HC(hipMemsetAsync(d_deleted, 0, S, st));
    {
      uint32_t *d_fl = A.get<uint32_t>("forb.list", E->forbidden.size());
      h2d(E, d_fl, E->forbidden.data(), 4 * E->forbidden.size());
      launch(st, k_mark_list, E->forbidden.size(), (const uint32_t *)d_fl, (uint64_t)E->forbidden.size(), d_forb);
    }
    for (const char *nm : {"el.holder_idx", "el.occ", "el.noov", "el.rep_pos"})
      HC(hipMemsetAsync(A.get<int32_t>(nm, S), 0xff, 4 * S, st));
    HC(hipMemsetAsync(A.get<uint8_t>("el.del", S), 0, S, st));
    sub_of = A.get<int32_t>("sub_of", S);
    HC(hipMemsetAsync(sub_of, 0xff, 4 * S, st));

    snap_join(E);
    E->snap_on = false;
    E->lc_snap_n = 0;
    E->csr_ready = false;
    E->log_on = fl->emit_substitution_log != 0;
    E->log_from.clear();
    E->log_key.clear();
    E->log_val.clear();
    E->log_ptr.assign(1, 0);
  }

  void eq_simplification() {
    load_wait(E, 0);
    eq_rep = A.get<int32_t>("eq_rep", S);
    HC(hipMemsetAsync(eq_rep, 0xff, 4 * S, st));
    {
      uint32_t *uf = A.get<uint32_t>("uf", S);
      uint32_t *cnt = A.get<uint32_t>("eq.cnt", S);
      int32_t *maxrow = A.get<int32_t>("eq.maxrow", S);
      uint32_t *minf = A.get<uint32_t>("eq.minf", S);
      uint32_t *minr = A.get<uint32_t>("eq.minr", S);
      uint8_t *in_eq = A.get<uint8_t>("eq.in", S);
      uint32_t *bf = A.get<uint32_t>("eq.bf", E->eq.n);
      uint32_t *bfn = A.get<uint32_t>("eq.bfn", 1);
      launch(st, k_iota_u32, S, uf, S);
      HC(hipMemsetAsync(cnt, 0, 4 * S, st));
      HC(hipMemsetAsync(maxrow, 0xff, 4 * S, st));
      HC(hipMemsetAsync(minf, 0xff, 4 * S, st));
      HC(hipMemsetAsync(minr, 0xff, 4 * S, st));
      HC(hipMemsetAsync(in_eq, 0, S, st));
      HC(hipMemsetAsync(bfn, 0, 4, st));
      if (E->eq.n) {
        launch(st, k_eq_union, E->eq.n, (const uint64_t *)E->eq.ptr, (const uint32_t *)E->eq.key, E->eq.n, uf, d_err);
        launch(st, k_eq_stats, E->eq.n, (const uint64_t *)E->eq.ptr, (const uint32_t *)E->eq.key, E->eq.n, uf,
               (const uint8_t *)d_forb, cnt, maxrow, minf, minr, in_eq);
// ... 230 lines not shown
    if (!keys_first) {
      load_wait(E, 2);
      if (lin.n) {
        kg1.run(st, 72 * E->lin.nnz + 20 * lin.n + 8 + 77 * E->lin.nnz + 16 * lin.n, [&] {
          launch(st, k_make_ragged, lin.n, E->F, (const uint64_t *)E->lin.ptr, (const uint32_t *)E->lin.key, (const Fe *)E->lin.val,
                 lin.n, (uint64_t)1, lin.off, lin.len, lin.key, lin.val);
          launch(st, k_linear_frames12, lin.n, E->F, lin, (const int32_t *)eq_rep, (const uint8_t *)ce_has, (const Fe *)ce_val);
        });
      }
    }
    if (g_prof_env) fprintf(stderr, "[rs-prof] linear rows: %s\n", keys_first ? "keys first" : "keys + values");
    HC(hipStreamSynchronize(st));
    E->stats.eq_ms = now_ms() - T0;
  }
  void linear_values() {
    load_wait(E, 2);
    kg1.run(st, 77 * E->lin.nnz + 20 * lin.n + 8, [&] {
      launch(st, k_lin_valframes, lin.n, E->F, (const uint64_t *)E->lin.ptr, (const uint32_t *)E->lin.key, (const Fe *)E->lin.val,
             lin.n, lin, (const int32_t *)eq_rep, (const uint8_t *)ce_has, (const Fe *)ce_val, (const uint8_t *)lin_fixed);
    });
  }

  void mk_in(rs_engine::Blk &B, DRows &R, const char *nm, hipStream_t ms) {
    R.n = B.n;
    R.off = A.get<uint64_t>(std::string(nm) + ".off", R.n);
    R.len = A.get<uint32_t>(std::string(nm) + ".len", R.n);
    R.key = A.get<uint32_t>(std::string(nm) + ".key", B.nnz);
    R.val = A.get<Fe>(std::string(nm) + ".val", B.nnz);
    if (R.n)
      kg1.run(ms, 72 * B.nnz + 20 * R.n + 8, [&] {
        launch(ms, k_make_ragged, R.n, E->F, (const uint64_t *)B.ptr, (const uint32_t *)B.key, (const Fe *)B.val, R.n, (uint64_t)0,
               R.off, R.len, R.key, R.val);
      });
  }
  void stage_nl() {
    if (nl_staged) return;
    load_wait(E, 3);
    static const bool on_main = env_flag("RS_NLC_MAIN");
    hipStream_t cs = on_main ? st : E->stc;
    rs_engine::Blk *blk[3] = {&E->na, &E->nb, &E->nc};
    const char *nm[3] = {"nla", "nlb", "nlc"};
    for (int q = 0; q < 3; ++q) mk_in(*blk[q], nl_in[q], nm[q], cs);
    HC(hipEventRecord(E->ev_nlc, cs));
    HC(hipStreamWaitEvent(st, E->ev_nlc, 0));
    nl_staged = true;
  }
  void heap_reserve(uint64_t need) {
    if (heap_top + need <= E->heap_cap && E->heap_k) return;
    uint64_t ncap = std::max<uint64_t>(heap_top + need + (heap_top + need) / 16, E->heap_cap + E->heap_cap / 4);
    ncap = std::max<uint64_t>(ncap, 1 << 16);
    uint32_t *nk = nullptr;
    Fe *nv = nullptr;
    HC(hipStreamSynchronize(st));
    HC(hipMalloc((void **)&nk, 4 * ncap));
    HC(hipMalloc((void **)&nv, 32 * ncap));
    if (heap_top) {
      HC(hipMemcpyAsync(nk, E->heap_k, 4 * heap_top, hipMemcpyDeviceToDevice, st));
      HC(hipMemcpyAsync(nv, E->heap_v, 32 * heap_top, hipMemcpyDeviceToDevice, st));
      HC(hipStreamSynchronize(st));
    }
    if (E->snap_on) HC(hipStreamSynchronize(E->stc));
    if (E->heap_k) { HC(hipFree(E->heap_k)); HC(hipFree(E->heap_v)); }
    E->heap_k = heap_k = nk;
    E->heap_v = heap_v = nv;
    E->heap_cap = ncap;
  }

  void setup_non_linear() {
    heap_top = 0;
    heap_k = E->heap_k;
    heap_v = E->heap_v;
    d_bytes = A.get<unsigned long long>("nl.bytes", 1);
    HC(hipMemsetAsync(d_bytes, 0, 8, st));
    d_fw_err = A.get<int>("fw.err", 1);
    HC(hipMemsetAsync(d_fw_err, 0, 4, st));
    fr.F = E->F;
    fr.eq_rep = eq_rep;
    fr.ce_has = ce_has;
    fr.ce_val = ce_val;
    fr.sub_of = sub_of;
    for (int q = 0; q < 3; ++q) {
      stor[q].n = n_nl;
      stor[q].off = A.get<uint64_t>(part_name("st.", q, ".off"), n_nl);
      stor[q].len = A.get<uint32_t>(part_name("st.", q, ".len"), n_nl);
    }
    if (n_nl) {
      for (int q = 0; q < 3; ++q) cap[q] = A.get<uint64_t>(part_name("nl.cap", q, ""), n_nl);
      cap3 = A.get<U3>("nl.c3", n_nl); sc3 = A.get<U3>("nl.s3", n_nl);
    }
  }

  void snap_views(const DRows (&src)[3], const char *pre, DRows (&cp)[3], ViewCopy &vc) {
    for (int q = 0; q < 3; ++q) {
      cp[q] = src[q];
      cp[q].off = vc.off[q] = A.get<uint64_t>(part_name(pre, q, ".off"), src[q].n);
      cp[q].len = vc.len[q] = A.get<uint32_t>(part_name(pre, q, ".len"), src[q].n);
    }
  }
  template <class G>
  void snap_tail(const uint64_t n[3], hipEvent_t *evs, const char *what, const char *when, G &&gather) {
    for (int q = 0; q < 3; ++q) {
      const uint64_t b = E->snap_e[q];
      const std::string xn = std::string("out.") + "abc"[q];
      uint32_t *col = A.get<uint32_t>(xn + ".xcol", 1);
      uint64_t *val = A.get<uint64_t>(xn + ".xval", 1);
      if (!n[q]) continue;
      gather(q, col, val, b);
      HC(hipEventRecord(evs[q], E->stc));
      snap_push(E, {(uint32_t *)E->snap_host[2 * q] + b, col + b, 4 * n[q], evs[q]});
      snap_push(E, {(uint64_t *)E->snap_host[2 * q + 1] + 4 * b, val + 4 * b, 32 * n[q], evs[q]});
      E->snap_e[q] = b + n[q];
    }
    HC(hipEventRecord(E->ev_snap, E->stc));
    if (g_prof_env)
      fprintf(stderr, "[rs-prof] stream: %s %llu / %llu / %llu entries (%.1f MB)%s\n", what, (unsigned long long)n[0],
              (unsigned long long)n[1], (unsigned long long)n[2], 36e-6 * (n[0] + n[1] + n[2]), when);
  }
  void snap_take(const uint64_t *late, uint64_t hi_rows) {
    if (!E->stream_out || !n_nl) return;
    so_early = A.get<uint8_t>("so.early", n_nl);
    so_eoff = A.get<U3>("so.eoff", n_nl);
    U3 *elen = A.get<U3>("so.elen", n_nl);
    Comm *CM = E->comm.get();
    const bool shard = CM && CM->world > 1;
    DRows cp[3];
    ViewCopy vc;
    snap_views(stor, "so.", cp, vc);
    launch(st, k_snap_flags, n_nl, stor[0], stor[1], stor[2], late, n_nl, shard ? E->nl_lo : (uint64_t)0, shard ? E->nl_hi : hi_rows, so_early, elen,
           vc);
    const U3 et = excl_scan_u3(E, elen, so_eoff, n_nl, "so");
    E->lc_snap_n = shard ? 0 : lc.n;
    E->lc_snap_base = et.c;
    const uint64_t lc_e = shard ? 0 : lc.top;
    const uint64_t ev[3] = {et.a, et.b, et.c + lc_e};
    E->sh_full = false;
    if (shard) {
      for (int q = 0; q < 3; ++q) E->sh_cap[q] = CM->max_u64(std::max<uint64_t>(ev[q] + ev[q] / 4 + 65536, E->sh_cap[q]), st);
      E->sh_ent = CM->shared_host(0, sh_ent_bytes(E), st);
      if (!E->sh_ent) {
        if (g_prof_env) fprintf(stderr, "[rs-prof] no shared host memory: unstreamed per-rank result\n");
        E->stream_out = false;
        return;
      }
    }
    HC(hipEventRecord(E->ev_snap0, st));
    HC(hipStreamWaitEvent(E->stc, E->ev_snap0, 0));
    for (int q = 0; q < 3; ++q) {
      E->snap_e[q] = 0;
      E->snap_hint[q] = std::max(E->snap_hint[q], ev[q]);
      const uint64_t est = hi_rows < n_nl && hi_rows ? (uint64_t)((double)ev[q] * n_nl / hi_rows) : ev[q];
      const uint64_t cap = std::max<uint64_t>(est + std::max<uint64_t>(est / 4, 1 << 16), E->snap_hint[q]);
      const std::string xn = std::string("out.") + "abc"[q];
      (void)A.get<uint32_t>(xn + ".xcol", cap);
      (void)A.get<uint64_t>(xn + ".xval", 4 * cap);
      E->snap_cap[q] = cap;
      E->snap_host[2 * q] = shard ? (void *)(sh_col(E, q) + CM->rank * E->sh_cap[q]) : pin_get(E, kPinCol + q, 4 * cap);
      E->snap_host[2 * q + 1] = shard ? (void *)(sh_val(E, q) + 4 * CM->rank * E->sh_cap[q]) : pin_get(E, kPinVal + q, 32 * cap);
    }
    snap_tail(ev, E->ev_snapq, "early region", late ? " after the first pass" : "", [&](int q, uint32_t *col, uint64_t *val, uint64_t) {
      E->kg[2].run(E->stc, 13 * n_nl + 72 * ev[q], [&] {
        launch(E->stc, k_snap_gather, n_nl, E->F, cp[q], (const uint8_t *)so_early, (const U3 *)so_eoff, q, n_nl, col, val,
               (const uint64_t *)nullptr, (uint64_t)0);
      });
      if (q == 2 && lc_e) {
        const DRows lcv = lc.view(A);
        E->kg[2].run(E->stc, 72 * lc_e, [&] {
          launch(E->stc, k_lc_snap, lc_e, E->F, (const uint32_t *)lcv.key, (const Fe *)lcv.val, lc_e, col + et.c, val + 4 * et.c);
        });
      }
    });
    E->snap_on = true;
  }
  void snap_take2() {
    if (!E->snap_on || !nl_late || !n_late || (E->comm && E->comm->world > 1)) return;
    HC(hipStreamWaitEvent(st, E->ev_snap, 0));
    U3 *elen = A.get<U3>("so.elen2", n_late), *eoff2 = A.get<U3>("so.eoff2", n_late);
    DRows cp[3];
    ViewCopy vc;
    snap_views(stor, "so2.", cp, vc);
    launch(st, k_snap_lens2_l, n_late, stor[0], stor[1], stor[2], (const uint32_t *)nl_lids, n_late, elen, vc);
    const U3 et = excl_scan_u3(E, elen, eoff2, n_late, "so2");
    const uint64_t e2[3] = {et.a, et.b, et.c};
    for (int q = 0; q < 3; ++q) E->snap_hint[q] = std::max(E->snap_hint[q], E->snap_e[q] + e2[q]);
    for (int q = 0; q < 3; ++q)
      if (E->snap_e[q] + e2[q] > E->snap_cap[q]) return;
    launch(st, k_snap_mark2_l, n_late, (const uint32_t *)nl_lids, (const U3 *)elen, (const U3 *)eoff2,
           U3{E->snap_e[0], E->snap_e[1], E->snap_e[2]}, n_late, so_early, so_eoff);
    HC(hipEventRecord(E->ev_snap0, st));
    HC(hipStreamWaitEvent(E->stc, E->ev_snap0, 0));
    snap_tail(e2, E->ev_snapq + 3, "second snapshot", "", [&](int q, uint32_t *col, uint64_t *val, uint64_t) {
      E->kg[2].run(E->stc, 28 * n_late + 72 * e2[q], [&] {
        launch(E->stc, k_snap_gather_l, n_late, E->F, cp[q], (const uint32_t *)nl_lids, (const U3 *)elen, (const U3 *)so_eoff, q, n_late,
               col, val);
      });
    });
  }
  void snap_take_h2(uint64_t h) {
    if (!E->snap_on || (E->comm && E->comm->world > 1)) return;
    HC(hipStreamWaitEvent(st, E->ev_snap, 0));
    U3 *elen = A.get<U3>("so.elenh", n_nl), *eoffh = A.get<U3>("so.eoffh", n_nl);
    DRows cp[3];
    ViewCopy vc;
    snap_views(stor, "soh.", cp, vc);
    launch(st, k_snap_lens_rng, n_nl, stor[0], stor[1], stor[2], (const uint64_t *)nl_late, h, n_nl, n_nl, elen, vc);
    const U3 et = excl_scan_u3(E, elen, eoffh, n_nl, "soh");
    const uint64_t e2[3] = {et.a, et.b, et.c};
    for (int q = 0; q < 3; ++q) E->snap_hint[q] = std::max(E->snap_hint[q], E->snap_e[q] + e2[q]);
    for (int q = 0; q < 3; ++q)
      if (E->snap_e[q] + e2[q] > E->snap_cap[q]) return;
    launch(st, k_snap_mark_sel, n_nl, (const U3 *)elen, (const U3 *)eoffh, U3{E->snap_e[0], E->snap_e[1], E->snap_e[2]}, n_nl,
           so_early, so_eoff);
    HC(hipEventRecord(E->ev_snap0, st));
    HC(hipStreamWaitEvent(E->stc, E->ev_snap0, 0));
    snap_tail(e2, E->ev_snaph, "the first pass's second half", "", [&](int q, uint32_t *col, uint64_t *val, uint64_t) {
      E->kg[2].run(E->stc, 13 * (n_nl - h) + 72 * e2[q], [&] {
        launch(E->stc, k_snap_gather, n_nl - h, E->F, cp[q], (const uint8_t *)so_early, (const U3 *)so_eoff, q, n_nl, col, val,
               (const uint64_t *)nullptr, h);
      });
    });
  }
  void nl_phase(int phase, const uint32_t *ids, uint64_t n, hipEvent_t e0, hipEvent_t e1, uint64_t split = ~0ull,
                const std::function<void()> &between = {}) {
    stage_nl();
    NLArgs a{};
    a.fr = fr;
    a.a = nl_in[0]; a.b = nl_in[1]; a.c = nl_in[2];
    a.cap_a = cap[0]; a.cap_b = cap[1]; a.cap_c = cap[2];
    a.bytes = d_bytes;
    a.ids = ids;
    a.n = n;
    a.phase = phase;
    a.hmark = hmark;
    a.late = nl_late;
    launch(st, k_nl_count, n, a);
    const bool lists = phase == 1 && n_nl;
    if (lists) {
      dev_scan_u64(E, nl_late, nl_lpos, n_nl, st, "nll");
      launch(st, k_scatter_ids, n_nl, (const uint64_t *)nl_late, (const uint64_t *)nl_lpos, n_nl, nl_lids);
    }
    launch(st, k_pack3, n, (const uint64_t *)cap[0], (const uint64_t *)cap[1], (const uint64_t *)cap[2], n, cap3);
    const U3 t3 = lists ? excl_scan_u3(E, cap3, sc3, n, "nl", nl_late + n_nl - 1, nl_lpos + n_nl - 1, &n_late)
                        : excl_scan_u3(E, cap3, sc3, n, "nl");
    if (g_prof_env) fprintf(stderr, "[rs-prof] nl phase %d: %llu rows, %llu heap entries\n", phase, (unsigned long long)n,
                            (unsigned long long)(t3.a + t3.b + t3.c));
    heap_reserve(t3.a + t3.b + t3.c);
    launch(st, k_set_offsets_u3, n, (const U3 *)sc3, heap_top, heap_top + t3.a, heap_top + t3.a + t3.b, n, stor[0].off, stor[1].off,
           stor[2].off, phase == 1 ? (const U3 *)cap3 : nullptr, ids);
    heap_top += t3.a + t3.b + t3.c;
    for (DRows &R : stor) { R.key = heap_k; R.val = heap_v; }
    a.oa = stor[0]; a.ob = stor[1]; a.oc = stor[2];
    FrameWaveArgs w{};
    w.fr = fr;
    for (int q = 0; q < 3; ++q) { w.in[q] = nl_in[q]; w.out[q] = stor[q]; w.cap[q] = cap[q]; }
    w.ids = ids;
    w.n = n;
    w.late = phase == 1 ? nl_late : nullptr;
    w.big = A.get<uint32_t>(phase == 1 ? "nl.big1" : "nl.big2", n);
    w.n_big = A.get<unsigned>(phase == 1 ? "nl.nbig1" : "nl.nbig2", 1);
    w.err = d_fw_err;
    w.bytes = d_bytes;
    HC(hipMemsetAsync(w.n_big, 0, 4, st));
#ifdef RS_FWCLK
    w.clk = A.get<unsigned long long>(phase == 1 ? "fw.clk1" : "fw.clk2", 32 + 8 * 64);
    HC(hipMemsetAsync(w.clk, 0, 8 * (32 + 8 * 64), st));
#endif
    a.xlist = w.big;
    a.n_xlist = w.n_big;
    HC(hipEventRecord(e0, st));
    fh_split = split < n;
    if (fh_split) {
      w.n = split;
      launch_capped(st, k_frames_wave<0>, split, kFwBlocks, w);
      launch(st, k_nl_fill, n, a);
      HC(hipEventRecord(E->ev_fh[0], st));
      between();
      HC(hipMemsetAsync(w.n_big, 0, 4, st));
      HC(hipEventRecord(E->ev_fh[1], st));
      w.x0 = split;
      w.n = n;
      launch_capped(st, k_frames_wave<0>, n - split, kFwBlocks, w);
    } else {
      launch_capped(st, k_frames_wave<0>, n, kFwBlocks, w);
    }
    launch(st, k_nl_fill, n, a);
    HC(hipEventRecord(e1, st));
    if (g_prof_env) {
      unsigned nb = 0;
      HC(hipMemcpyAsync(&nb, w.n_big, 4, hipMemcpyDeviceToHost, st));
      HC(hipStreamSynchronize(st));
      fprintf(stderr, "[rs-prof] nl phase %d: %u rows over a wave batch\n", phase, nb);
      if (w.clk) {
        unsigned long long c[32 + 8 * 64];
        HC(hipMemcpy(c, w.clk, sizeof c, hipMemcpyDeviceToHost));
        fprintf(stderr, "[rs-prof] frames clocks (Mcycles summed over waves): groups %.1f entries %.1f terms %.1f rank %.1f "
                "heads %.1f emit %.1f rows %.1f plan %.1f | batches %llu, wave total %.1f over %llu waves\n",
                c[0] / 1e6, c[1] / 1e6, c[2] / 1e6, c[3] / 1e6, c[4] / 1e6, c[5] / 1e6, c[6] / 1e6, c[7] / 1e6, c[8],
                c[9] / 1e6, c[10]);
        fprintf(stderr, "[rs-prof] frames fallbacks: A const %llu, B const %llu | emit: loads %.1f values %.1f sync %.1f stores %.1f\n",
                c[12], c[13], c[16] / 1e6, c[17] / 1e6, c[18] / 1e6, c[19] / 1e6);
      }
    }
    E->stats.apply_kernel_launches++;
  }
  void nl_ms(hipEvent_t e0, hipEvent_t e1) {
    float ms = 0;
    HC(hipEventSynchronize(e1));
    if (fh_split) {
      float m2 = 0;
      HC(hipEventElapsedTime(&ms, e0, E->ev_fh[0]));
      HC(hipEventElapsedTime(&m2, E->ev_fh[1], e1));
      ms += m2;
      fh_split = false;
    } else {
      HC(hipEventElapsedTime(&ms, e0, e1));
    }
    E->stats.apply_kernel_ms += ms;
  }
  void head_overlap(const uint32_t *ids, uint64_t n_head, const ElimArgs &ea) {
    hmark = A.get<uint8_t>("nl.hmark", E->S);
    nl_late = A.get<uint64_t>("nl.late", n_nl);
    nl_lpos = A.get<uint64_t>("nl.lpos", n_nl);
    nl_lids = A.get<uint32_t>("nl.lids", n_nl);
    HC(hipMemsetAsync(hmark, 0, E->S, st));
    hipLaunchKernelGGL(k_mark_head_keys, dim3(16, (unsigned)n_head), dim3(256), 0, st, ea.rows, (const uint32_t *)ea.perm,
                       (const uint64_t *)ea.cl_off, ids, hmark);
    HC(hipGetLastError());
    fr.h_off = ea.h_off; fr.h_len = ea.h_len; fr.pk = ea.pk; fr.pv = ea.pv;
    const bool halves = E->stream_out && !(E->comm && E->comm->world > 1) &&
                        n_nl >= env_u64("RS_HALVES_MIN", 1ull << 20, 0, UINT64_MAX) && !env_flag("RS_NO_HALVES");
    const double frac = env_f64("RS_HALF_FRAC", 0.5, 0.0, 1.0);
    const uint64_t h = halves ? std::max<uint64_t>(1, std::min<uint64_t>(n_nl - 1, (uint64_t)(n_nl * frac))) : n_nl;
    nl_phase(1, nullptr, n_nl, E->ev[kEvNl0], E->ev[kEvNl1], h, [&] { snap_take(nl_late, h); });
    if (!halves) snap_take(nl_late, n_nl);
    else snap_take_h2(h);
    nl_split = true;
  }

  void linear_round1() {
    P = get_pool(E, 1 << 20);
    const HeadOverlap overlap = [this](const uint32_t *ids, uint64_t n_head, const ElimArgs &ea) { head_overlap(ids, n_head, ea); };
    const std::function<void()> values = [this] { linear_values(); };
    if (apply_linear) {
      uint8_t *relevant = nullptr;
      if (E->comm && E->comm->world > 1 && !E->log_on) {
        relevant = A.get<uint8_t>("x.relevant", S);
        HC(hipMemsetAsync(relevant, 0, S, st));
        if (n_nl) {
          stage_nl();
          for (const DRows &R : nl_in)
            launch(st, k_mark_relevant, R.n, R,(const int32_t *)eq_rep, (const uint8_t *)ce_has, relevant);
        }
      }
      if (E->comm && E->comm->world > 1) load_order_collectives(E);
      run_linear_simplification(E, lin, fl->use_old_heuristics, eo, P, d_err, d_forb, sub_of, d_deleted,
                                n_nl ? &overlap : nullptr, keys_first ? &values : nullptr, relevant);
      if (E->log_on) log_linear_round(E, eo, P);
      collect_leftovers(E, eo, P, lc);
      E->stats.rounds++;
    } else {
      if (!keys_first) lc.append(E, lin, nullptr, lin.n);
      else throw RsError(RS_E_INTERNAL, "--O1 with keys-first linear rows");
    }
  }

  void non_linear_frames() {
    double Ts = now_ms();
    fr.h_off = A.get<uint64_t>("el.h_off", 1);
    fr.h_len = A.get<uint32_t>("el.h_len", 1);
    fr.pk = P.pk;
    fr.pv = P.pv;
    if (n_nl) {
      if (nl_split) nl_ms(E->ev[kEvNl0], E->ev[kEvNl1]);
      if (!nl_split) {
        nl_phase(0, nullptr, n_nl, E->ev[kEvFill0], E->ev[kEvFill1]);
        snap_take(nullptr, n_nl);
        nl_ms(E->ev[kEvFill0], E->ev[kEvFill1]);
      } else if (n_late) {
        nl_phase(2, nl_lids, n_late, E->ev[kEvFill0], E->ev[kEvFill1]);
        snap_take2();
        nl_ms(E->ev[kEvFill0], E->ev[kEvFill1]);
      }
    }
    unsigned long long bytes = 0;
    HC(hipMemcpyAsync(&bytes, d_bytes, 8, hipMemcpyDeviceToHost, st));
    st_ids = A.get<uint32_t>("st.ids", n_nl);
    wl_ids = A.get<uint32_t>("wl.ids", n_nl);
    uint64_t *h_wl = (uint64_t *)pin_get(E, kPinRead, kPinRb);
    if (n_nl) {
      uint64_t *fl_lin = A.get<uint64_t>("fl.lin", n_nl), *p_lin = A.get<uint64_t>("fl.plin", n_nl);
      uint64_t *d_wl = A.get<uint64_t>("fl.tot", 1);
      launch(st, k_flag_lin, n_nl, (const uint32_t *)stor[0].len, (const uint32_t *)stor[1].len, n_nl, fl_lin);
      dev_scan_u64(E, fl_lin, p_lin, n_nl, st, "fl");
      launch(st, k_scan_total_u64, 1, (const uint64_t *)fl_lin, (const uint64_t *)p_lin, n_nl, d_wl);
      launch(st, k_split_ids, n_nl, (const uint64_t *)fl_lin, (const uint64_t *)p_lin, n_nl, wl_ids, st_ids);
      HC(hipMemcpyAsync(h_wl, d_wl, 8, hipMemcpyDeviceToHost, st));
    }
    HC(hipStreamSynchronize(st));
    if (n_nl) {
      n_wl = h_wl[0];
      if (n_wl > n_nl) throw RsError(RS_E_INTERNAL, "non-linear split: row counts out of range");
      n_st = n_nl - n_wl;
    }
    E->stats.apply_bytes += bytes;
    if (no_rounds > 0) no_rounds--;

    for (int q = 0; q < 3; ++q) {
      sv[q].n = n_st;
      sv[q].key = heap_k;
      sv[q].val = heap_v;
      sv[q].off = A.get<uint64_t>(part_name("sv.", q, ".off"), n_st);
      sv[q].len = A.get<uint32_t>(part_name("sv.", q, ".len"), n_st);
    }
    lv.n = n_wl;
    lv.key = heap_k;
    lv.val = heap_v;
    lv.off = A.get<uint64_t>("lv.off", n_wl);
    lv.len = A.get<uint32_t>("lv.len", n_wl);
    if (n_st + n_wl)
      launch(st, k_view_rows4, n_st + n_wl, stor[0], stor[1], stor[2], (const uint32_t *)st_ids, n_st, (const uint32_t *)wl_ids, n_wl,
             sv[0], sv[1], sv[2], lv);
    nlmap = A.get<uint8_t>("nlmap", S);
    HC(hipMemsetAsync(nlmap, 0, S, st));
    if (n_st) launch(st, k_mark_keys3, n_st, sv[0], sv[1], sv[2], n_st, nlmap);
    HC(hipStreamSynchronize(st));
    E->stats.subst_ms += now_ms() - Ts;
    E->stats.nl_ms += now_ms() - Ts;
  }

  void snap_round(const uint8_t *touched, const int32_t *turn) {
    if (!so_dirty || !n_st || (E->comm && E->comm->world > 1)) return;
    HC(hipStreamWaitEvent(st, E->ev_snap, 0));
    U3 *elen = A.get<U3>("so.rlen", n_st), *eoff3 = A.get<U3>("so.roff", n_st);
    DRows cp[3];
    ViewCopy vc;
    snap_views(sv, "sor.", cp, vc);
    launch(st, k_snap_lens_round, n_st, sv[0], sv[1], sv[2], touched, turn, (const uint32_t *)st_ids, (const uint8_t *)so_early, n_st, elen, vc);
    const U3 et = excl_scan_u3(E, elen, eoff3, n_st, "sor");
    const uint64_t e3[3] = {et.a, et.b, et.c};
    if (!(e3[0] | e3[1] | e3[2])) return;
    for (int q = 0; q < 3; ++q) E->snap_hint[q] = std::max(E->snap_hint[q], E->snap_e[q] + e3[q]);
    for (int q = 0; q < 3; ++q)
      if (E->snap_e[q] + e3[q] > E->snap_cap[q]) return;
    launch(st, k_snap_mark_round, n_st, (const uint32_t *)st_ids, (const U3 *)elen, (const U3 *)eoff3,
           U3{E->snap_e[0], E->snap_e[1], E->snap_e[2]}, n_st, so_early, so_eoff, so_dirty);
    HC(hipEventRecord(E->ev_snap0, st));
    HC(hipStreamWaitEvent(E->stc, E->ev_snap0, 0));
    snap_tail(e3, E->ev_snapq + 3, "round snapshot", "", [&](int q, uint32_t *col, uint64_t *val, uint64_t b) {
      E->kg[2].run(E->stc, 24 * n_st + 72 * e3[q], [&] {
        launch(E->stc, k_snap_gather_st, n_st, E->F, cp[q], (const U3 *)elen, (const U3 *)eoff3, b, q, n_st, col, val);
      });
    });
  }

  void rounds() {
    apply_round = apply_linear && no_rounds > 0 && n_wl > 0;
    if (so_early) {
      so_dirty = A.get<uint8_t>("so.dirty", n_st ? n_st : 1);
      if (n_st) HC(hipMemsetAsync(so_dirty, 0, n_st, st));
    }
    if (env_flag("RS_DEBUG")) {
      HC(hipStreamSynchronize(st));
      fprintf(stderr, "[rs-debug] heap %p cap %llu top %llu n_st %llu n_wl %llu\n", (void *)heap_k,
              (unsigned long long)E->heap_cap, (unsigned long long)heap_top, (unsigned long long)n_st, (unsigned long long)n_wl);
      for (uint64_t r = 0; r < std::min<uint64_t>(n_st, 3); ++r) {
        uint64_t o = 0; uint32_t l = 0;
        HC(hipMemcpy(&o, sv[2].off + r, 8, hipMemcpyDeviceToHost));
        HC(hipMemcpy(&l, sv[2].len + r, 4, hipMemcpyDeviceToHost));
        std::vector<uint32_t> kk; std::vector<Fe> vv;
        d2h_row(E, sv[2], r, kk, vv);
        fprintf(stderr, "[rs-debug]  st %llu C off %llu len %u:", (unsigned long long)r, (unsigned long long)o, l);
        for (size_t i = 0; i < kk.size(); ++i) fprintf(stderr, " %u:%llu", kk[i], (unsigned long long)ffrom_mont(E->F, vv[i]).l[0]);
        fprintf(stderr, "\n");
      }
    }
    if (apply_round) {
      double Tm = now_ms();
      for (int q = 0; q < 3; ++q) {
        m0[q] = sv[q];
        m0[q].off = A.get<uint64_t>(part_name("m0.", q, ".off"), n_st);
        m0[q].len = A.get<uint32_t>(part_name("m0.", q, ".len"), n_st);
      }
      if (n_st)
        for (int q = 0; q < 3; ++q) {
          HC(hipMemcpyAsync(m0[q].off, sv[q].off, 8 * n_st, hipMemcpyDeviceToDevice, st));
          HC(hipMemcpyAsync(m0[q].len, sv[q].len, 4 * n_st, hipMemcpyDeviceToDevice, st));
        }
      qflag = A.get<uint8_t>("m.qflag", S);
      HC(hipMemsetAsync(qflag, 0, S, st));
      E->stats.subst_ms += now_ms() - Tm;
      E->stats.map_ms += now_ms() - Tm;
      rank_of = A.get<int32_t>("rank_of", S);
      HC(hipMemsetAsync(rank_of, 0xff, 4 * S, st));
      r_sub_of = A.get<int32_t>("r.sub_of", S);
      HC(hipMemsetAsync(r_sub_of, 0xff, 4 * S, st));
      while (apply_round) round_once();
    }
  }
  void query_initial(const std::vector<uint32_t> &sigs) {
    auto &minit = ML.minit;
    std::vector<uint32_t> q;
// ... 686 lines not shown
```

include/rs_simplify.h:

```cpp
#ifndef RS_SIMPLIFY_H
#define RS_SIMPLIFY_H

#include <stdint.h>

#ifdef __cplusplus
extern "C" {
#endif

#define RS_ABI_VERSION 14

enum rs_status {
  RS_OK = 0,
  RS_E_INVALID = -1,
  RS_E_OOM_DEVICE = -2,
  RS_E_HIP = -3,
  RS_E_RCCL = -4,
  RS_E_INTERNAL = -5,
  RS_E_NODEVICE = -6
};

enum rs_prime {
  RS_PRIME_BN128 = 0,
  RS_PRIME_BLS12381 = 1,
  RS_PRIME_GOLDILOCKS = 2,
  RS_PRIME_GRUMPKIN = 3,
  RS_PRIME_PALLAS = 4,
  RS_PRIME_VESTA = 5,
  RS_PRIME_SECQ256R1 = 6,
  RS_PRIME_BLS12377 = 7,
  RS_PRIME_CUSTOM = 255
};

typedef struct rs_lc {
  uint64_t n_rows;
  uint64_t nnz;
  uint64_t *ptr;
  uint32_t *col;
  uint64_t *val;
} rs_lc;

typedef struct rs_input {
  uint32_t prime_id;
  uint64_t prime[4];
  uint64_t max_signal;
  uint64_t n_pub_out;
  uint64_t n_pub_in;
  uint64_t n_priv_in;
  uint64_t n_forbidden;
  uint32_t *forbidden;
  rs_lc cons_eq;
  rs_lc eq;
  rs_lc linear;
  rs_lc nl_a;
  rs_lc nl_b;
  rs_lc nl_c;
} rs_input;

typedef struct rs_flags {
  uint32_t flag_s;
  uint32_t use_old_heuristics;
  uint64_t no_rounds;
  uint32_t emit_substitution_log;
// ... 83 lines not shown
  uint64_t round_fill_bytes;
  uint64_t round_fill_launches;
  uint64_t alg_bytes;
  double h2d_wait_ms;
  double d2h_ms;
  double host_total_ms;
  double write_ms;
  double tail_fin_ms;
  uint64_t tail_fin_bytes;
  uint64_t tail_fin_launches;
  double head_fin_ms;
  uint64_t head_fin_bytes;
  uint64_t head_fin_launches;
  double small_ms;
  uint64_t small_bytes;
  uint64_t small_launches;
  double prep_ms;
  uint64_t prep_launches;
  double cluster_dev_ms;
  uint64_t cluster_bytes;
  uint64_t cluster_launches;
  double giant_ms;
  uint64_t giant_bytes;
  uint64_t giant_launches;
  uint64_t giant_merges;
  double check_ms;
  uint64_t check_bytes;
  uint64_t check_launches;
  double ragged_ms;
  uint64_t ragged_bytes;
  uint64_t ragged_launches;
  double gather_ms;
  uint64_t gather_bytes;
  uint64_t gather_launches;
  double cluster_host_ms;
  double read_ms;
  double read_upload_ms;
  double read_kernel_ms;
  double read_d2h_ms;
  double sym_write_ms;
  double sym_in_ms;
  double sym_kernel_ms;
  double sym_out_ms;
} rs_stats;

typedef struct rs_json_stats {
  double write_ms;
  double in_ms;
  double kernel_ms;
  double out_ms;
  uint64_t bytes;
} rs_json_stats;

typedef struct rs_engine rs_engine;

const char *rs_last_error(void);
int rs_abi_version(void);

int rs_simplify(const rs_input *in, const rs_flags *fl, rs_output **out);
void rs_output_free(rs_output *out);

int rs_engine_create(int device, rs_engine **eng);
int rs_engine_load(rs_engine *eng, const rs_input *in);
int rs_engine_run(rs_engine *eng, const rs_flags *fl);
int rs_engine_fetch(rs_engine *eng, rs_output **out);
int rs_engine_stats(rs_engine *eng, rs_stats *st);
void rs_engine_destroy(rs_engine *eng);

int rs_engine_simplify(rs_engine *eng, const rs_input *in, const rs_flags *fl, const rs_output **out);

int rs_engine_write_r1cs(rs_engine *eng, const char *path, const char *o0_r1cs);

void *rs_host_alloc(uint64_t bytes);
void rs_host_free(void *p);

#define RS_COMM_ID_BYTES 128
typedef struct rs_group rs_group;
int rs_comm_unique_id(uint8_t id[RS_COMM_ID_BYTES]);
int rs_engine_join_rccl(rs_engine *eng, int world, int rank, const uint8_t id[RS_COMM_ID_BYTES]);
rs_group *rs_group_create(int world);
int rs_engine_join_group(rs_engine *eng, rs_group *g, int rank);
void rs_group_destroy(rs_group *g);
int rs_simplify_multi(const rs_input *in, const rs_flags *fl, int n_devices, const int *devices, rs_output **out);
int rs_engine_join_host(rs_engine *eng, int world, int rank, const char *tag);

int rs_engine_inject_fault(rs_engine *eng, int where);

int rs_read_r1cs_o0(const char *path, rs_input **in);
void rs_input_free(rs_input *in);
int rs_engine_read_r1cs_o0(rs_engine *eng, const char *path, const rs_input **in);
int rs_read_r1cs_o0_device(int device, const char *path, rs_input **in);
int rs_write_r1cs(const char *path, const rs_input *in, const rs_output *out);
int rs_write_r1cs_gates(const char *path, const rs_input *in, const rs_output *out, const char *o0_r1cs);
int rs_write_sym(const char *o0_sym, const char *path, const rs_output *out);
int rs_engine_write_sym(rs_engine *eng, const char *o0_sym, const char *path);
int rs_write_sym_device(int device, const char *o0_sym, const char *path, const rs_output *out);
int rs_write_constraints_json(const char *path, const rs_output *out);
int rs_write_substitution_json(const char *path, const rs_output *out);
int rs_engine_write_constraints_json(rs_engine *eng, const char *path);
int rs_engine_write_substitution_json(rs_engine *eng, const char *path);
int rs_write_constraints_json_device(int device, const char *path, const rs_output *out);
int rs_write_substitution_json_device(int device, const char *path, const rs_output *out);
int rs_engine_json_stats(rs_engine *eng, rs_json_stats *st);

typedef struct rs_witness {
  uint32_t prime_id;
  uint64_t prime[4];
  uint32_t n8;
  uint64_t n;
  uint64_t *val;
} rs_witness;

#define RS_WIT_INPUT 1u
#define RS_WIT_OUTPUT 2u
#define RS_WIT_LOG 4u
enum rs_witness_class {
  RS_WITC_CONS_EQ = 0,
  RS_WITC_EQ = 1,
  RS_WITC_LINEAR = 2,
  RS_WITC_NONLINEAR = 3,
  RS_WITC_OUTPUT = 4,
  RS_WITC_LOG = 5,
  RS_WITC_COUNT = 6
};
typedef struct rs_witness_report {
  uint64_t checked[6], failed[6], first_failed[6];
  double in_ms, kernel_ms, total_ms;
} rs_witness_report;

int rs_read_wtns(const char *path, rs_witness **w);
void rs_witness_free(rs_witness *w);
int rs_write_wtns(const char *path, const rs_witness *w, const rs_output *out);
int rs_check_witness(const rs_input *in, const rs_output *out, const rs_witness *w, uint32_t what, rs_witness_report *rep);
int rs_engine_load_witness(rs_engine *eng, const rs_witness *w);
int rs_engine_load_wtns(rs_engine *eng, const char *path);
int rs_engine_check_witness(rs_engine *eng, const rs_input *in, uint32_t what, rs_witness_report *rep);
int rs_engine_write_wtns(rs_engine *eng, const char *path);

typedef struct rs_lift_report {
  uint64_t n_labels, n_wires;
  uint64_t lifted;
  uint64_t free_labels;
  uint64_t shadowed;
  uint64_t levels;
  uint64_t entries;
  double in_ms, kernel_ms, total_ms;
} rs_lift_report;
int rs_lift_witness(const rs_output *out, const rs_witness *v, rs_witness **w, rs_lift_report *rep);
int rs_lift_witness_device(int device, const rs_output *out, const rs_witness *v, rs_witness **w, rs_lift_report *rep);
int rs_engine_lift_witness(rs_engine *eng, rs_lift_report *rep);
int rs_engine_fetch_witness(rs_engine *eng, rs_witness **w);
int rs_engine_write_wtns_resident(rs_engine *eng, const char *path);

int rs_synth(uint32_t kind, uint64_t rows, uint64_t seed, uint32_t prime_id, rs_input **in);

typedef struct rs_dag {
// ... 24 lines not shown
```

integration/rust/src/lib.rs:

```rust
#![allow(non_camel_case_types)]
use std::os::raw::{c_char, c_int, c_void};

pub const RS_ABI_VERSION: c_int = 14;
pub const RS_COMM_ID_BYTES: usize = 128;

pub const RS_OK: c_int = 0;
pub const RS_E_INVALID: c_int = -1;
pub const RS_E_OOM_DEVICE: c_int = -2;
pub const RS_E_HIP: c_int = -3;
pub const RS_E_RCCL: c_int = -4;
pub const RS_E_INTERNAL: c_int = -5;
pub const RS_E_NODEVICE: c_int = -6;

#[repr(C)]
#[derive(Clone, Copy)]
pub struct rs_lc {
    pub n_rows: u64,
    pub nnz: u64,
    pub ptr: *mut u64,
    pub col: *mut u32,
    pub val: *mut u64,
}

#[repr(C)]
pub struct rs_input {
    pub prime_id: u32,
    pub prime: [u64; 4],
    pub max_signal: u64,
    pub n_pub_out: u64,
    pub n_pub_in: u64,
    pub n_priv_in: u64,
    pub n_forbidden: u64,
    pub forbidden: *mut u32,
    pub cons_eq: rs_lc,
    pub eq: rs_lc,
    pub linear: rs_lc,
    pub nl_a: rs_lc,
    pub nl_b: rs_lc,
    pub nl_c: rs_lc,
}

#[repr(C)]
pub struct rs_flags {
    pub flag_s: u32,
    pub use_old_heuristics: u32,
    pub no_rounds: u64,
    pub emit_substitution_log: u32,
    pub device: i32,
}

#[repr(C)]
pub struct rs_output {
    pub n_constraints: u64,
    pub a: rs_lc,
    pub b: rs_lc,
    pub c: rs_lc,
// ... 114 lines not shown
    pub head_main_ms: f64,
    pub head_main_bytes: u64,
    pub head_launches: u64,
    pub tail_main_ms: f64,
    pub tail_main_bytes: u64,
    pub tail_launches: u64,
    pub round_fill_ms: f64,
    pub round_fill_bytes: u64,
    pub round_fill_launches: u64,
    pub alg_bytes: u64,
    pub h2d_wait_ms: f64,
    pub d2h_ms: f64,
    pub host_total_ms: f64,
    pub write_ms: f64,
    pub tail_fin_ms: f64,
    pub tail_fin_bytes: u64,
    pub tail_fin_launches: u64,
    pub head_fin_ms: f64,
    pub head_fin_bytes: u64,
    pub head_fin_launches: u64,
    pub small_ms: f64,
    pub small_bytes: u64,
    pub small_launches: u64,
    pub prep_ms: f64,
    pub prep_launches: u64,
    pub cluster_dev_ms: f64,
    pub cluster_bytes: u64,
    pub cluster_launches: u64,
    pub giant_ms: f64,
    pub giant_bytes: u64,
    pub giant_launches: u64,
    pub giant_merges: u64,
    pub check_ms: f64,
    pub check_bytes: u64,
    pub check_launches: u64,
    pub ragged_ms: f64,
    pub ragged_bytes: u64,
    pub ragged_launches: u64,
    pub gather_ms: f64,
    pub gather_bytes: u64,
    pub gather_launches: u64,
    pub cluster_host_ms: f64,
    pub read_ms: f64,
    pub read_upload_ms: f64,
    pub read_kernel_ms: f64,
    pub read_d2h_ms: f64,
    pub sym_write_ms: f64,
    pub sym_in_ms: f64,
    pub sym_kernel_ms: f64,
    pub sym_out_ms: f64,
}

#[repr(C)]
pub struct rs_witness {
    pub prime_id: u32,
    pub prime: [u64; 4],
    pub n8: u32,
    pub n: u64,
    pub val: *mut u64,
}

pub const RS_WIT_INPUT: u32 = 1;
pub const RS_WIT_OUTPUT: u32 = 2;
pub const RS_WIT_LOG: u32 = 4;
pub const RS_WITC_CONS_EQ: usize = 0;
pub const RS_WITC_EQ: usize = 1;
pub const RS_WITC_LINEAR: usize = 2;
pub const RS_WITC_NONLINEAR: usize = 3;
pub const RS_WITC_OUTPUT: usize = 4;
pub const RS_WITC_LOG: usize = 5;

#[repr(C)]
pub struct rs_witness_report {
    pub checked: [u64; 6],
    pub failed: [u64; 6],
    pub first_failed: [u64; 6],
    pub in_ms: f64,
    pub kernel_ms: f64,
    pub total_ms: f64,
}

#[repr(C)]
pub struct rs_lift_report {
    pub n_labels: u64,
    pub n_wires: u64,
    pub lifted: u64,
    pub free_labels: u64,
    pub shadowed: u64,
    pub levels: u64,
    pub entries: u64,
    pub in_ms: f64,
    pub kernel_ms: f64,
    pub total_ms: f64,
}

#[repr(C)]
pub struct rs_json_stats {
    pub write_ms: f64,
    pub in_ms: f64,
    pub kernel_ms: f64,
    pub out_ms: f64,
    pub bytes: u64,
}

#[repr(C)]
pub struct rs_engine {
    _private: [u8; 0],
}
#[repr(C)]
pub struct rs_group {
    _private: [u8; 0],
}

extern "C" {
    pub fn rs_last_error() -> *const c_char;
    pub fn rs_abi_version() -> c_int;
    pub fn rs_simplify(inp: *const rs_input, fl: *const rs_flags, out: *mut *mut rs_output) -> c_int;
    pub fn rs_output_free(out: *mut rs_output);
    pub fn rs_engine_create(device: c_int, eng: *mut *mut rs_engine) -> c_int;
    pub fn rs_engine_load(eng: *mut rs_engine, inp: *const rs_input) -> c_int;
    pub fn rs_engine_run(eng: *mut rs_engine, fl: *const rs_flags) -> c_int;
    pub fn rs_engine_fetch(eng: *mut rs_engine, out: *mut *mut rs_output) -> c_int;
    pub fn rs_engine_stats(eng: *mut rs_engine, st: *mut rs_stats) -> c_int;
    pub fn rs_engine_destroy(eng: *mut rs_engine);
    pub fn rs_engine_simplify(eng: *mut rs_engine, inp: *const rs_input, fl: *const rs_flags, out: *mut *const rs_output) -> c_int;
    pub fn rs_engine_write_r1cs(eng: *mut rs_engine, path: *const c_char, o0_r1cs: *const c_char) -> c_int;
    pub fn rs_host_alloc(bytes: u64) -> *mut c_void;
    pub fn rs_host_free(p: *mut c_void);
    pub fn rs_comm_unique_id(id: *mut u8) -> c_int;
    pub fn rs_engine_join_rccl(eng: *mut rs_engine, world: c_int, rank: c_int, id: *const u8) -> c_int;
    pub fn rs_group_create(world: c_int) -> *mut rs_group;
    pub fn rs_engine_join_group(eng: *mut rs_engine, g: *mut rs_group, rank: c_int) -> c_int;
    pub fn rs_group_destroy(g: *mut rs_group);
    pub fn rs_simplify_multi(inp: *const rs_input, fl: *const rs_flags, n_devices: c_int, devices: *const c_int, out: *mut *mut rs_output) -> c_int;
    pub fn rs_engine_join_host(eng: *mut rs_engine, world: c_int, rank: c_int, tag: *const c_char) -> c_int;
    pub fn rs_engine_inject_fault(eng: *mut rs_engine, where_: c_int) -> c_int;
    pub fn rs_read_r1cs_o0(path: *const c_char, inp: *mut *mut rs_input) -> c_int;
    pub fn rs_input_free(inp: *mut rs_input);
    pub fn rs_engine_read_r1cs_o0(eng: *mut rs_engine, path: *const c_char, inp: *mut *const rs_input) -> c_int;
    pub fn rs_read_r1cs_o0_device(device: c_int, path: *const c_char, inp: *mut *mut rs_input) -> c_int;
    pub fn rs_write_r1cs(path: *const c_char, inp: *const rs_input, out: *const rs_output) -> c_int;
    pub fn rs_write_r1cs_gates(path: *const c_char, inp: *const rs_input, out: *const rs_output, o0_r1cs: *const c_char) -> c_int;
    pub fn rs_write_sym(o0_sym: *const c_char, path: *const c_char, out: *const rs_output) -> c_int;
    pub fn rs_engine_write_sym(eng: *mut rs_engine, o0_sym: *const c_char, path: *const c_char) -> c_int;
    pub fn rs_write_sym_device(device: c_int, o0_sym: *const c_char, path: *const c_char, out: *const rs_output) -> c_int;
    pub fn rs_write_constraints_json(path: *const c_char, out: *const rs_output) -> c_int;
    pub fn rs_write_substitution_json(path: *const c_char, out: *const rs_output) -> c_int;
    pub fn rs_engine_write_constraints_json(eng: *mut rs_engine, path: *const c_char) -> c_int;
    pub fn rs_engine_write_substitution_json(eng: *mut rs_engine, path: *const c_char) -> c_int;
    pub fn rs_write_constraints_json_device(device: c_int, path: *const c_char, out: *const rs_output) -> c_int;
    pub fn rs_write_substitution_json_device(device: c_int, path: *const c_char, out: *const rs_output) -> c_int;
    pub fn rs_engine_json_stats(eng: *mut rs_engine, st: *mut rs_json_stats) -> c_int;
    pub fn rs_read_wtns(path: *const c_char, w: *mut *mut rs_witness) -> c_int;
    pub fn rs_witness_free(w: *mut rs_witness);
    pub fn rs_write_wtns(path: *const c_char, w: *const rs_witness, out: *const rs_output) -> c_int;
    pub fn rs_check_witness(inp: *const rs_input, out: *const rs_output, w: *const rs_witness, what: u32, rep: *mut rs_witness_report) -> c_int;
    pub fn rs_engine_load_witness(eng: *mut rs_engine, w: *const rs_witness) -> c_int;
    pub fn rs_engine_load_wtns(eng: *mut rs_engine, path: *const c_char) -> c_int;
    pub fn rs_engine_check_witness(eng: *mut rs_engine, inp: *const rs_input, what: u32, rep: *mut rs_witness_report) -> c_int;
    pub fn rs_engine_write_wtns(eng: *mut rs_engine, path: *const c_char) -> c_int;
    pub fn rs_lift_witness(out: *const rs_output, v: *const rs_witness, w: *mut *mut rs_witness, rep: *mut rs_lift_report) -> c_int;
    pub fn rs_lift_witness_device(device: c_int, out: *const rs_output, v: *const rs_witness, w: *mut *mut rs_witness, rep: *mut rs_lift_report) -> c_int;
    pub fn rs_engine_lift_witness(eng: *mut rs_engine, rep: *mut rs_lift_report) -> c_int;
    pub fn rs_engine_fetch_witness(eng: *mut rs_engine, w: *mut *mut rs_witness) -> c_int;
    pub fn rs_engine_write_wtns_resident(eng: *mut rs_engine, path: *const c_char) -> c_int;
    pub fn rs_synth(kind: u32, rows: u64, seed: u64, prime_id: u32, inp: *mut *mut rs_input) -> c_int;
    pub fn rs_flatten_dag(device: c_int, dag: *const rs_dag, inp: *mut *mut rs_input) -> c_int;
    pub fn rs_engine_flatten_dag(eng: *mut rs_engine, dag: *const rs_dag, inp: *mut *const rs_input) -> c_int;
}
```

Before: 239.5 million.

## Split non-linear pass into dependency levels overlapping head and tail elimination

Replaces the halves-based split of the non-linear frame pass with a three-level classification: each row is leveled by whether it touches keys from head clusters (2), the first tail group (1), or neither (0). Level-0 rows are processed in K slices on a side stream concurrently with elimination, level-1 rows once the first tail group is known, and only level-2 rows remain after linear elimination. It also builds level row lists via scan, adds per-pass snapshot/stream-out events, and exposes new nl_stats for diagnostics. The aim is more work overlapped with linear elimination, at the cost of extra classification kernels, scans, host syncs and more complex stream ordering.

After: 241.4 million (median of 6 runs). Within noise of the previous version (+0.8%).

```diff
diff --git a/circom_cvm_amd/abi.py b/circom_cvm_amd/abi.py
--- a/circom_cvm_amd/abi.py
+++ b/circom_cvm_amd/abi.py
@@ -124,6 +124,15 @@
 
     def as_dict(self):
         return {k: getattr(self, k) for k, _ in self._fields_}
+
+
+class RsNlStats(C.Structure):
+    _fields_ = [("nl_level_rows", C.c_uint64 * 3), ("nl_levels", C.c_uint64), ("nl_slices", C.c_uint64),
+                ("nl_pass_start_ms", C.c_double * 4), ("nl_pass_dev_ms", C.c_double * 4)]
+
+    def as_dict(self):
+        return {k: list(getattr(self, k)) if isinstance(getattr(self, k), C.Array) else getattr(self, k)
+                for k, _ in self._fields_}
 
 
 class RsJsonStats(C.Structure):
@@ -224,6 +233,7 @@
     ("rs_write_constraints_json_device", C.c_int, [C.c_int, C.c_char_p, C.POINTER(RsOutput)]),
     ("rs_write_substitution_json_device", C.c_int, [C.c_int, C.c_char_p, C.POINTER(RsOutput)]),
     ("rs_engine_json_stats", C.c_int, [C.c_void_p, C.POINTER(RsJsonStats)]),
+    ("rs_engine_nl_stats", C.c_int, [C.c_void_p, C.POINTER(RsNlStats)]),
     ("rs_read_wtns", C.c_int, [C.c_char_p, C.POINTER(C.POINTER(RsWitness))]),
     ("rs_witness_free", None, [C.POINTER(RsWitness)]),
     ("rs_write_wtns", C.c_int, [C.c_char_p, C.POINTER(RsWitness), C.POINTER(RsOutput)]),
@@ -408,6 +418,11 @@
     def write_wtns_resident(self, path: str):
         check(lib().rs_engine_write_wtns_resident(self._h, path.encode()))
 
+    def nl_stats(self) -> RsNlStats:
+        s = RsNlStats()
+        check(lib().rs_engine_nl_stats(self._h, C.byref(s)))
+        return s
+
     def json_stats(self) -> RsJsonStats:
         s = RsJsonStats()
         check(lib().rs_engine_json_stats(self._h, C.byref(s)))
diff --git a/circom_cvm_amd/csrc/engine.hip b/circom_cvm_amd/csrc/engine.hip
--- a/circom_cvm_amd/csrc/engine.hip
+++ b/circom_cvm_amd/csrc/engine.hip
@@ -211,6 +211,7 @@
   kEvNl0, kEvNl1,
   kEvCount
 };
+constexpr int kMaxSlices = 8, kMaxPass = kMaxSlices + 2;
 enum PinSlot {
   kPinPtr = 0,
   kPinCol = 3,
@@ -256,6 +257,7 @@
   uint64_t n_wires = 0, npiw = 0;
   rs_stats stats{};
   rs_json_stats jstats{};
+  rs_nl_stats nlst{};
   bool wit_on = false;
   uint64_t wit_n = 0;
   uint32_t wit_n8 = 0, wit_prime_id = 0;
@@ -304,11 +306,12 @@
     size_t bytes;
     hipEvent_t ready;
   };
-  hipEvent_t ev_snapq[6] = {};
-  hipEvent_t ev_snaph[3] = {};
+  hipEvent_t ev_snapq[3 * (kMaxPass + 1)] = {};
   double asm_t0_ms = 0, asm_end_ms = 0, snap_last_ms = 0;
   int snap_open = 0, asm_open = 0;
-  hipEvent_t ev_fh[2] = {};
+  hipEvent_t ev_pass[kMaxPass][2] = {};
+  hipEvent_t ev_l0 = nullptr;
+  hipEvent_t ev_t0 = nullptr;
   hipEvent_t ev_nlc = nullptr;
   std::mutex snap_m;
   std::condition_variable snap_cv;
@@ -605,19 +608,20 @@
   __host__ __device__ U3 operator()(const U3 &x, const U3 &y) const { return U3{x.a + y.a, x.b + y.b, x.c + y.c}; }
 };
 static U3 excl_scan_u3(rs_engine *E, const U3 *in, U3 *out, uint64_t n, const char *tag, const uint64_t *x_in = nullptr,
-                       const uint64_t *x_out = nullptr, uint64_t *x_sum = nullptr) {
+                       const uint64_t *x_out = nullptr, uint64_t *x_sum = nullptr, hipStream_t s = nullptr) {
   if (n == 0 && !x_sum) return U3{0, 0, 0};
+  if (!s) s = E->st;
   uint64_t *h = (uint64_t *)pin_get(E, kPinRead, kPinRb) + 8;
   if (n) {
-    excl_scan(E->A, std::string("scan3.tmp.") + tag, E->st, in, out, U3{0, 0, 0}, n, U3Plus());
-    HC(hipMemcpyAsync(h, in + n - 1, sizeof(U3), hipMemcpyDeviceToHost, E->st));
-    HC(hipMemcpyAsync(h + 3, out + n - 1, sizeof(U3), hipMemcpyDeviceToHost, E->st));
+    excl_scan(E->A, std::string("scan3.tmp.") + tag, s, in, out, U3{0, 0, 0}, n, U3Plus());
+    HC(hipMemcpyAsync(h, in + n - 1, sizeof(U3), hipMemcpyDeviceToHost, s));
+    HC(hipMemcpyAsync(h + 3, out + n - 1, sizeof(U3), hipMemcpyDeviceToHost, s));
   }
   if (x_sum) {
-    HC(hipMemcpyAsync(h + 6, x_in, 8, hipMemcpyDeviceToHost, E->st));
-    HC(hipMemcpyAsync(h + 7, x_out, 8, hipMemcpyDeviceToHost, E->st));
-  }
-  HC(hipStreamSynchronize(E->st));
+    HC(hipMemcpyAsync(h + 6, x_in, 8, hipMemcpyDeviceToHost, s));
+    HC(hipMemcpyAsync(h + 7, x_out, 8, hipMemcpyDeviceToHost, s));
+  }
+  HC(hipStreamSynchronize(s));
   if (x_sum) *x_sum = h[6] + h[7];
   return n ? U3{h[0] + h[3], h[1] + h[4], h[2] + h[5]} : U3{0, 0, 0};
 }
@@ -1503,7 +1507,7 @@
   HC(hipGetLastError());
 }
 
-using HeadOverlap = std::function<void(const uint32_t *head_ids, uint64_t n_head, const ElimArgs &a)>;
+using HeadOverlap = std::function<void(const uint32_t *head_ids, uint64_t n_head, uint64_t n_t1, const ElimArgs &a)>;
 
 static void run_linear_simplification(rs_engine *E, const DRows &view, int old_heur, ElimOut &eo, Pool &P,
                                       int *d_err, uint8_t *d_forb, int32_t *sub_of, uint8_t *deleted,
@@ -1715,9 +1719,11 @@
       HC(hipEventRecord(E->ev_sm[1], E->ste));
       HC(hipEventRecord(E->ev[kEvLane], E->st));
       n_tgroups = 0;
+      uint64_t n_t1 = 0;
       if (n_tail) {
-        static const uint64_t split = env_u64("RS_TAIL_SPLIT", kTailSplit, 1, UINT64_MAX / 2);
-        const uint64_t n_t1 = n_tail > split + split / 4 ? split : n_tail, n_t2 = n_tail - n_t1;
+        const uint64_t split = env_u64("RS_TAIL_SPLIT", kTailSplit, 1, UINT64_MAX / 2);
+        n_t1 = n_tail > split + split / 4 ? split : n_tail;
+        const uint64_t n_t2 = n_tail - n_t1;
         n_tgroups = n_t2 ? 2 : 1;
         auto tail_group = [&](hipStream_t s, ElimArgs g, const uint32_t *ids, uint64_t n, const char *cls_name, int grp) {
           const bool timed = grp == 0;
@@ -1803,7 +1809,7 @@
           ao.pk = G.pk;
           ao.pv = G.pv;
         }
-        (*overlap)(d_big, n_head, ao);
+        (*overlap)(d_big, n_head, n_t1, ao);
       }
       if (n_head) HC(hipStreamWaitEvent(E->st, E->ev[kEvHeadEnd], 0));
       HC(hipEventRecord(E->ev[kEvElim1], E->st));
@@ -2544,8 +2550,10 @@
     HC(hipEventCreateWithFlags(&E->ev_snap0, hipEventDisableTiming));
     for (auto &ev : E->ev_chunk) HC(hipEventCreateWithFlags(&ev, hipEventDisableTiming));
     for (auto &ev : E->ev_snapq) HC(hipEventCreateWithFlags(&ev, hipEventDisableTiming));
-    for (auto &ev : E->ev_snaph) HC(hipEventCreateWithFlags(&ev, hipEventDisableTiming));
-    for (auto &ev : E->ev_fh) HC(hipEventCreate(&ev));
+    for (auto &pe : E->ev_pass)
+      for (auto &ev : pe) HC(hipEventCreate(&ev));
+    HC(hipEventCreateWithFlags(&E->ev_l0, hipEventDisableTiming));
+    HC(hipEventCreate(&E->ev_t0));
     HC(hipEventCreateWithFlags(&E->ev_nlc, hipEventDisableTiming));
     *eng = E.release();
     return RS_OK;
@@ -2599,6 +2607,11 @@
     if (ev) (void)hipEventDestroy(ev);
   for (auto &ev : E->ev_snapq)
     if (ev) (void)hipEventDestroy(ev);
+  for (auto &pe : E->ev_pass)
+    for (auto &ev : pe)
+      if (ev) (void)hipEventDestroy(ev);
+  if (E->ev_l0) (void)hipEventDestroy(E->ev_l0);
+  if (E->ev_t0) (void)hipEventDestroy(E->ev_t0);
   if (E->heap_k) (void)hipFree(E->heap_k);
   if (E->heap_v) (void)hipFree(E->heap_v);
   if (E->st) (void)hipStreamDestroy(E->st);
@@ -3106,6 +3119,12 @@
   });
 }
 
+int rs_engine_nl_stats(rs_engine *E, rs_nl_stats *st) {
+  if (!E || !st) { set_error("rs_engine_nl_stats: null argument"); return RS_E_INVALID; }
+  *st = E->nlst;
+  return RS_OK;
+}
+
 int rs_engine_json_stats(rs_engine *E, rs_json_stats *st) {
   if (!E || !st) { set_error("rs_engine_json_stats: null argument"); return RS_E_INVALID; }
   *st = E->jstats;
diff --git a/circom_cvm_amd/csrc/frames_wave.hpp b/circom_cvm_amd/csrc/frames_wave.hpp
--- a/circom_cvm_amd/csrc/frames_wave.hpp
+++ b/circom_cvm_amd/csrc/frames_wave.hpp
@@ -29,7 +29,6 @@
   int cap_by_row;
   const uint32_t *ids;
   uint64_t n;
-  uint64_t x0;
   const uint64_t *late;
   uint32_t *big;
   unsigned *n_big;
@@ -692,7 +691,7 @@
 #endif
   const uint64_t nw = (uint64_t)gridDim.x * kFwWaves;
   uint32_t fx_n = 0, fx_terms = 0;
-  for (uint64_t base = A.x0 + ((uint64_t)blockIdx.x * kFwWaves + wv) * 64; base < A.n; base += nw * 64) {
+  for (uint64_t base = ((uint64_t)blockIdx.x * kFwWaves + wv) * 64; base < A.n; base += nw * 64) {
     const uint64_t x = base + lane;
     bool act = x < A.n;
     uint64_t r = 0, ioff[3] = {0, 0, 0}, ooff[3] = {0, 0, 0};
diff --git a/circom_cvm_amd/csrc/kernels.hpp b/circom_cvm_amd/csrc/kernels.hpp
--- a/circom_cvm_amd/csrc/kernels.hpp
+++ b/circom_cvm_amd/csrc/kernels.hpp
@@ -2997,7 +2997,7 @@
 };
 
 __global__ void k_mark_head_keys(DRows rows, const uint32_t *perm, const uint64_t *cl_off, const uint32_t *ids,
-                                 uint8_t *hmark) {
+                                 uint8_t *hmark, uint8_t v) {
   const uint32_t c = ids[blockIdx.y];
   const uint64_t b = cl_off[c], e = cl_off[c + 1];
   for (uint64_t i = b + blockIdx.x * blockDim.x + threadIdx.x; i < e; i += (uint64_t)gridDim.x * blockDim.x) {
@@ -3005,8 +3005,58 @@
     const uint64_t o = rows.off[r];
     for (uint32_t j = 0; j < rows.len[r]; ++j) {
       const uint32_t k = rows.key[o + j];
-      if (k) hmark[k] = 1;
-    }
+      if (k) hmark[k] = v;
+    }
+  }
+}
+
+__device__ inline uint32_t d_part_level(const FrameArgs &F, const uint8_t *hmark, const DRows &R, uint64_t r) {
+  const uint64_t o = R.off[r];
+  uint32_t lv = 0;
+  for (uint32_t i = 0; i < R.len[r]; ++i) {
+    const uint32_t k = R.key[o + i];
+    const int32_t t = F.eq_rep ? F.eq_rep[k] : -1;
+    const uint32_t k1 = t >= 0 ? (uint32_t)t : k;
+    if (F.ce_has && F.ce_has[k1]) continue;
+    lv = lv > hmark[k1] ? lv : hmark[k1];
+  }
+  return lv;
+}
+__global__ void k_nl_levels(FrameArgs fr, const uint8_t *hmark, DRows a, DRows b, DRows c, uint64_t n, uint8_t *lvl,
+                            uint64_t *flag3) {
+  for (uint64_t r = gtid(); r < n; r += gstride()) {
+    uint32_t lv = d_part_level(fr, hmark, a, r);
+    const uint32_t lb = d_part_level(fr, hmark, b, r), lc = d_part_level(fr, hmark, c, r);
+    lv = lv > lb ? lv : lb;
+    lv = lv > lc ? lv : lc;
+    lv = lv > 2 ? 2 : lv;
+    lvl[r] = (uint8_t)lv;
+    flag3[3 * r + 0] = lv == 0;
+    flag3[3 * r + 1] = lv == 1;
+    flag3[3 * r + 2] = lv == 2;
+  }
+}
+__global__ void k_level_lists(const uint8_t *lvl, const uint64_t *pos3, uint64_t base1, uint64_t base2, uint64_t n,
+                              uint32_t *lids) {
+  for (uint64_t r = gtid(); r < n; r += gstride()) {
+    const uint32_t l = lvl[r];
+    lids[(l == 0 ? 0 : (l == 1 ? base1 : base2)) + pos3[3 * r + l]] = (uint32_t)r;
+  }
+}
+__global__ void k_level_entries(const uint8_t *lvl, const uint32_t *la, const uint32_t *lb, const uint32_t *lc, uint64_t n,
+                                unsigned long long *cnt) {
+  unsigned long long w[3] = {0, 0, 0};
+  for (uint64_t r = gtid(); r < n; r += gstride()) {
+    if ((la[r] | lb[r]) == 0) continue;
+    const unsigned long long e = (unsigned long long)la[r] + lb[r] + lc[r];
+#pragma unroll
+    for (uint32_t l = 0; l < 3; ++l) w[l] += lvl[r] == l ? e : 0;
+  }
+#pragma unroll
+  for (int q = 0; q < 3; ++q) {
+#pragma unroll
+    for (int d = 32; d >= 1; d >>= 1) w[q] += __shfl_xor(w[q], d);
+    if ((threadIdx.x & 63) == 0 && w[q]) atomicAdd(cnt + q, w[q]);
   }
 }
 
diff --git a/circom_cvm_amd/csrc/output.hpp b/circom_cvm_amd/csrc/output.hpp
--- a/circom_cvm_amd/csrc/output.hpp
+++ b/circom_cvm_amd/csrc/output.hpp
@@ -46,25 +46,9 @@
   }
 }
 
-__global__ void k_snap_lens_rng(DRows a, DRows b, DRows c, const uint64_t *late, uint64_t lo, uint64_t hi, uint64_t n, U3 *elen,
-                                ViewCopy vc) {
-  for (uint64_t i = gtid(); i < n; i += gstride()) {
-    const bool ok = i >= lo && i < hi && !(late && late[i]) && (a.len[i] | b.len[i]) != 0;
-    elen[i] = ok ? U3{a.len[i], b.len[i], c.len[i]} : U3{0, 0, 0};
-    if (ok) view_copy(vc, a, b, c, i, a.len[i], b.len[i], c.len[i]);
-  }
-}
-__global__ void k_snap_mark_sel(const U3 *elen, const U3 *eoff2, U3 base, uint64_t n, uint8_t *early, U3 *eoff) {
-  for (uint64_t i = gtid(); i < n; i += gstride()) {
-    if ((elen[i].a | elen[i].b) == 0) continue;
-    early[i] = 1;
-    eoff[i] = U3{base.a + eoff2[i].a, base.b + eoff2[i].b, base.c + eoff2[i].c};
-  }
-}
-
 __global__ void k_snap_gather(FieldP F, DRows R, const uint8_t *early, const U3 *eoff, int q, uint64_t n, uint32_t *col,
-                              uint64_t *val, const uint64_t *only, uint64_t lo) {
-  for (uint64_t r = lo + gtid(); r < n; r += gstride()) {
+                              uint64_t *val, const uint64_t *only) {
+  for (uint64_t r = gtid(); r < n; r += gstride()) {
     if (!early[r] || (only && !only[r])) continue;
     const uint64_t o = u3_sel(eoff[r], q), s = R.off[r];
     const uint32_t len = R.len[r];
diff --git a/circom_cvm_amd/csrc/run.hpp b/circom_cvm_amd/csrc/run.hpp
--- a/circom_cvm_amd/csrc/run.hpp
+++ b/circom_cvm_amd/csrc/run.hpp
@@ -36,11 +36,16 @@
   uint64_t *cap[3] = {};
   U3 *cap3 = nullptr, *sc3 = nullptr;
   uint64_t *nl_late = nullptr, *nl_lpos = nullptr;
-  uint8_t *hmark = nullptr;
+  uint8_t *hmark = nullptr, *nl_lvl = nullptr;
   uint32_t *nl_lids = nullptr;
   uint64_t n_late = 0;
+  bool nl_listed = false;
+  uint64_t lvl_n[3] = {0, 0, 0};
+  int n_pass = 0;
+  int n_timed = 0;
+  int pass_slot[kMaxPass] = {};
+  double pass_host_ms = 0;
   bool nl_split = false;
-  bool fh_split = false;
   uint8_t *so_early = nullptr;
   U3 *so_eoff = nullptr;
   uint8_t *so_dirty = nullptr;
@@ -69,6 +74,7 @@
 
   void init() {
     E->stats = rs_stats{};
+    E->nlst = rs_nl_stats{};
     E->stats.world = E->comm ? (uint64_t)E->comm->world : 1;
     for (int g = 1; g < 3; ++g) {
       E->kg[g].n = 0;
@@ -81,6 +87,7 @@
       E->A.flush();
     }
     T0 = now_ms();
+    HC(hipEventRecord(E->ev_t0, st));
     d_err = A.get<int>("err", 1);
     HC(hipMemsetAsync(d_err, 0, 4, st));
 
@@ -417,6 +424,7 @@
     uint32_t *nk = nullptr;
     Fe *nv = nullptr;
     HC(hipStreamSynchronize(st));
+    if (nl_listed) HC(hipStreamSynchronize(E->ste));
     HC(hipMalloc((void **)&nk, 4 * ncap));
     HC(hipMalloc((void **)&nv, 32 * ncap));
     if (heap_top) {
@@ -453,6 +461,11 @@
       for (int q = 0; q < 3; ++q) cap[q] = A.get<uint64_t>(part_name("nl.cap", q, ""), n_nl);
       cap3 = A.get<U3>("nl.c3", n_nl); sc3 = A.get<U3>("nl.s3", n_nl);
     }
+    if (E->stream_out && n_nl) {
+      so_early = A.get<uint8_t>("so.early", n_nl);
+      so_eoff = A.get<U3>("so.eoff", n_nl);
+      HC(hipMemsetAsync(so_early, 0, n_nl, st));
+    }
   }
 
   void snap_views(const DRows (&src)[3], const char *pre, DRows (&cp)[3], ViewCopy &vc) {
@@ -481,7 +494,7 @@
       fprintf(stderr, "[rs-prof] stream: %s %llu / %llu / %llu entries (%.1f MB)%s\n", what, (unsigned long long)n[0],
               (unsigned long long)n[1], (unsigned long long)n[2], 36e-6 * (n[0] + n[1] + n[2]), when);
   }
-  void snap_take(const uint64_t *late, uint64_t hi_rows) {
+  void snap_take(const uint64_t *late) {
     if (!E->stream_out || !n_nl) return;
     so_early = A.get<uint8_t>("so.early", n_nl);
     so_eoff = A.get<U3>("so.eoff", n_nl);
@@ -491,7 +504,7 @@
     DRows cp[3];
     ViewCopy vc;
     snap_views(stor, "so.", cp, vc);
-    launch(st, k_snap_flags, n_nl, stor[0], stor[1], stor[2], late, n_nl, shard ? E->nl_lo : (uint64_t)0, shard ? E->nl_hi : hi_rows, so_early, elen,
+    launch(st, k_snap_flags, n_nl, stor[0], stor[1], stor[2], late, n_nl, shard ? E->nl_lo : (uint64_t)0, shard ? E->nl_hi : n_nl, so_early, elen,
            vc);
     const U3 et = excl_scan_u3(E, elen, so_eoff, n_nl, "so");
     E->lc_snap_n = shard ? 0 : lc.n;
@@ -513,8 +526,7 @@
     for (int q = 0; q < 3; ++q) {
       E->snap_e[q] = 0;
       E->snap_hint[q] = std::max(E->snap_hint[q], ev[q]);
-      const uint64_t est = hi_rows < n_nl && hi_rows ? (uint64_t)((double)ev[q] * n_nl / hi_rows) : ev[q];
-      const uint64_t cap = std::max<uint64_t>(est + std::max<uint64_t>(est / 4, 1 << 16), E->snap_hint[q]);
+      const uint64_t cap = std::max<uint64_t>(ev[q] + std::max<uint64_t>(ev[q] / 4, 1 << 16), E->snap_hint[q]);
       const std::string xn = std::string("out.") + "abc"[q];
       (void)A.get<uint32_t>(xn + ".xcol", cap);
       (void)A.get<uint64_t>(xn + ".xval", 4 * cap);
@@ -525,7 +537,7 @@
     snap_tail(ev, E->ev_snapq, "early region", late ? " after the first pass" : "", [&](int q, uint32_t *col, uint64_t *val, uint64_t) {
       E->kg[2].run(E->stc, 13 * n_nl + 72 * ev[q], [&] {
         launch(E->stc, k_snap_gather, n_nl, E->F, cp[q], (const uint8_t *)so_early, (const U3 *)so_eoff, q, n_nl, col, val,
-               (const uint64_t *)nullptr, (uint64_t)0);
+               (const uint64_t *)nullptr);
       });
       if (q == 2 && lc_e) {
         const DRows lcv = lc.view(A);
@@ -536,123 +548,114 @@
     });
     E->snap_on = true;
   }
-  void snap_take2() {
-    if (!E->snap_on || !nl_late || !n_late || (E->comm && E->comm->world > 1)) return;
-    HC(hipStreamWaitEvent(st, E->ev_snap, 0));
-    U3 *elen = A.get<U3>("so.elen2", n_late), *eoff2 = A.get<U3>("so.eoff2", n_late);
+  void snap_list(const uint32_t *ids, uint64_t n, uint64_t x0, hipStream_t s, int p, const char *what) {
+    if (!E->stream_out || !so_early || !n) return;
+    U3 *elen = A.get<U3>("so.elen2", n_nl) + x0, *eoff2 = A.get<U3>("so.eoff2", n_nl) + x0;
     DRows cp[3];
     ViewCopy vc;
     snap_views(stor, "so2.", cp, vc);
-    launch(st, k_snap_lens2_l, n_late, stor[0], stor[1], stor[2], (const uint32_t *)nl_lids, n_late, elen, vc);
-    const U3 et = excl_scan_u3(E, elen, eoff2, n_late, "so2");
+    launch(s, k_snap_lens2_l, n, stor[0], stor[1], stor[2], ids, n, elen, vc);
+    const U3 et = excl_scan_u3(E, elen, eoff2, n, "so2", nullptr, nullptr, nullptr, s);
     const uint64_t e2[3] = {et.a, et.b, et.c};
-    for (int q = 0; q < 3; ++q) E->snap_hint[q] = std::max(E->snap_hint[q], E->snap_e[q] + e2[q]);
+    uint64_t lc_e = 0;
+    if (!E->snap_on) {
+      E->lc_snap_n = lc.n;
+      E->lc_snap_base = et.c;
+      lc_e = lc.top;
+      E->sh_full = false;
+      for (int q = 0; q < 3; ++q) {
+        const uint64_t x = q == 2 ? lc_e : 0;
+        const uint64_t est = std::max<uint64_t>((uint64_t)((double)e2[q] * ((double)n_nl / (double)n)), e2[q]) + x;
+        const uint64_t cap = std::max<uint64_t>(est + std::max<uint64_t>(est / 4, 1 << 16), E->snap_hint[q]);
+        const std::string xn = std::string("out.") + "abc"[q];
+        (void)A.get<uint32_t>(xn + ".xcol", cap);
+        (void)A.get<uint64_t>(xn + ".xval", 4 * cap);
+        E->snap_e[q] = 0;
+        E->snap_cap[q] = cap;
+        E->snap_host[2 * q] = pin_get(E, kPinCol + q, 4 * cap);
+        E->snap_host[2 * q + 1] = pin_get(E, kPinVal + q, 32 * cap);
+      }
+      E->snap_on = true;
+    }
+    const uint64_t add[3] = {e2[0], e2[1], e2[2] + lc_e};
+    for (int q = 0; q < 3; ++q) E->snap_hint[q] = std::max(E->snap_hint[q], E->snap_e[q] + add[q]);
     for (int q = 0; q < 3; ++q)
-      if (E->snap_e[q] + e2[q] > E->snap_cap[q]) return;
-    launch(st, k_snap_mark2_l, n_late, (const uint32_t *)nl_lids, (const U3 *)elen, (const U3 *)eoff2,
-           U3{E->snap_e[0], E->snap_e[1], E->snap_e[2]}, n_late, so_early, so_eoff);
-    HC(hipEventRecord(E->ev_snap0, st));
+      if (E->snap_e[q] + add[q] > E->snap_cap[q]) return;
+    launch(s, k_snap_mark2_l, n, ids, (const U3 *)elen, (const U3 *)eoff2, U3{E->snap_e[0], E->snap_e[1], E->snap_e[2]}, n,
+           so_early, so_eoff);
+    HC(hipEventRecord(E->ev_snap0, s));
     HC(hipStreamWaitEvent(E->stc, E->ev_snap0, 0));
-    snap_tail(e2, E->ev_snapq + 3, "second snapshot", "", [&](int q, uint32_t *col, uint64_t *val, uint64_t) {
-      E->kg[2].run(E->stc, 28 * n_late + 72 * e2[q], [&] {
-        launch(E->stc, k_snap_gather_l, n_late, E->F, cp[q], (const uint32_t *)nl_lids, (const U3 *)elen, (const U3 *)so_eoff, q, n_late,
-               col, val);
-      });
+    snap_tail(add, E->ev_snapq + 3 * p, what, "", [&](int q, uint32_t *col, uint64_t *val, uint64_t b) {
+      if (e2[q])
+        E->kg[2].run(E->stc, 28 * n + 72 * e2[q], [&] {
+          launch(E->stc, k_snap_gather_l, n, E->F, cp[q], ids, (const U3 *)elen, (const U3 *)so_eoff, q, n, col, val);
+        });
+      if (q == 2 && lc_e) {
+        const DRows lcv = lc.view(A);
+        E->kg[2].run(E->stc, 72 * lc_e, [&] {
+          launch(E->stc, k_lc_snap, lc_e, E->F, (const uint32_t *)lcv.key, (const Fe *)lcv.val, lc_e, col + b + e2[2],
+                 val + 4 * (b + e2[2]));
+        });
+      }
     });
   }
-  void snap_take_h2(uint64_t h) {
-    if (!E->snap_on || (E->comm && E->comm->world > 1)) return;
-    HC(hipStreamWaitEvent(st, E->ev_snap, 0));
-    U3 *elen = A.get<U3>("so.elenh", n_nl), *eoffh = A.get<U3>("so.eoffh", n_nl);
-    DRows cp[3];
-    ViewCopy vc;
-    snap_views(stor, "soh.", cp, vc);
-    launch(st, k_snap_lens_rng, n_nl, stor[0], stor[1], stor[2], (const uint64_t *)nl_late, h, n_nl, n_nl, elen, vc);
-    const U3 et = excl_scan_u3(E, elen, eoffh, n_nl, "soh");
-    const uint64_t e2[3] = {et.a, et.b, et.c};
-    for (int q = 0; q < 3; ++q) E->snap_hint[q] = std::max(E->snap_hint[q], E->snap_e[q] + e2[q]);
-    for (int q = 0; q < 3; ++q)
-      if (E->snap_e[q] + e2[q] > E->snap_cap[q]) return;
-    launch(st, k_snap_mark_sel, n_nl, (const U3 *)elen, (const U3 *)eoffh, U3{E->snap_e[0], E->snap_e[1], E->snap_e[2]}, n_nl,
-           so_early, so_eoff);
-    HC(hipEventRecord(E->ev_snap0, st));
-    HC(hipStreamWaitEvent(E->stc, E->ev_snap0, 0));
-    snap_tail(e2, E->ev_snaph, "the first pass's second half", "", [&](int q, uint32_t *col, uint64_t *val, uint64_t) {
-      E->kg[2].run(E->stc, 13 * (n_nl - h) + 72 * e2[q], [&] {
-        launch(E->stc, k_snap_gather, n_nl - h, E->F, cp[q], (const uint8_t *)so_early, (const U3 *)so_eoff, q, n_nl, col, val,
-               (const uint64_t *)nullptr, h);
-      });
-    });
-  }
-  void nl_phase(int phase, const uint32_t *ids, uint64_t n, hipEvent_t e0, hipEvent_t e1, uint64_t split = ~0ull,
-                const std::function<void()> &between = {}) {
+  void nl_phase(int phase, const uint32_t *ids, uint64_t n, hipEvent_t e0, hipEvent_t e1, hipStream_t s = nullptr,
+                uint64_t x0 = 0, int slot = 0) {
+    if (!s) s = st;
     stage_nl();
     NLArgs a{};
     a.fr = fr;
     a.a = nl_in[0]; a.b = nl_in[1]; a.c = nl_in[2];
-    a.cap_a = cap[0]; a.cap_b = cap[1]; a.cap_c = cap[2];
+    a.cap_a = cap[0] + x0; a.cap_b = cap[1] + x0; a.cap_c = cap[2] + x0;
     a.bytes = d_bytes;
     a.ids = ids;
     a.n = n;
     a.phase = phase;
     a.hmark = hmark;
     a.late = nl_late;
-    launch(st, k_nl_count, n, a);
+    pass_host_ms = now_ms() - T0;
+    launch(s, k_nl_count, n, a);
     const bool lists = phase == 1 && n_nl;
     if (lists) {
-      dev_scan_u64(E, nl_late, nl_lpos, n_nl, st, "nll");
-      launch(st, k_scatter_ids, n_nl, (const uint64_t *)nl_late, (const uint64_t *)nl_lpos, n_nl, nl_lids);
-    }
-    launch(st, k_pack3, n, (const uint64_t *)cap[0], (const uint64_t *)cap[1], (const uint64_t *)cap[2], n, cap3);
-    const U3 t3 = lists ? excl_scan_u3(E, cap3, sc3, n, "nl", nl_late + n_nl - 1, nl_lpos + n_nl - 1, &n_late)
-                        : excl_scan_u3(E, cap3, sc3, n, "nl");
+      dev_scan_u64(E, nl_late, nl_lpos, n_nl, s, "nll");
+      launch(s, k_scatter_ids, n_nl, (const uint64_t *)nl_late, (const uint64_t *)nl_lpos, n_nl, nl_lids);
+    }
+    launch(s, k_pack3, n, (const uint64_t *)a.cap_a, (const uint64_t *)a.cap_b, (const uint64_t *)a.cap_c, n, cap3 + x0);
+    const U3 t3 = lists ? excl_scan_u3(E, cap3, sc3, n, "nl", nl_late + n_nl - 1, nl_lpos + n_nl - 1, &n_late, s)
+                        : excl_scan_u3(E, cap3 + x0, sc3 + x0, n, "nl", nullptr, nullptr, nullptr, s);
     if (g_prof_env) fprintf(stderr, "[rs-prof] nl phase %d: %llu rows, %llu heap entries\n", phase, (unsigned long long)n,
                             (unsigned long long)(t3.a + t3.b + t3.c));
     heap_reserve(t3.a + t3.b + t3.c);
-    launch(st, k_set_offsets_u3, n, (const U3 *)sc3, heap_top, heap_top + t3.a, heap_top + t3.a + t3.b, n, stor[0].off, stor[1].off,
-           stor[2].off, phase == 1 ? (const U3 *)cap3 : nullptr, ids);
+    launch(s, k_set_offsets_u3, n, (const U3 *)(sc3 + x0), heap_top, heap_top + t3.a, heap_top + t3.a + t3.b, n, stor[0].off,
+           stor[1].off, stor[2].off, phase == 1 ? (const U3 *)cap3 : nullptr, ids);
     heap_top += t3.a + t3.b + t3.c;
     for (DRows &R : stor) { R.key = heap_k; R.val = heap_v; }
     a.oa = stor[0]; a.ob = stor[1]; a.oc = stor[2];
     FrameWaveArgs w{};
     w.fr = fr;
-    for (int q = 0; q < 3; ++q) { w.in[q] = nl_in[q]; w.out[q] = stor[q]; w.cap[q] = cap[q]; }
+    for (int q = 0; q < 3; ++q) { w.in[q] = nl_in[q]; w.out[q] = stor[q]; w.cap[q] = cap[q] + x0; }
     w.ids = ids;
     w.n = n;
     w.late = phase == 1 ? nl_late : nullptr;
-    w.big = A.get<uint32_t>(phase == 1 ? "nl.big1" : "nl.big2", n);
-    w.n_big = A.get<unsigned>(phase == 1 ? "nl.nbig1" : "nl.nbig2", 1);
+    w.big = A.get<uint32_t>(phase == 1 ? "nl.big1" : "nl.big2", n_nl) + x0;
+    w.n_big = A.get<unsigned>(phase == 1 ? "nl.nbig1" : "nl.nbig2", kMaxPass) + slot;
     w.err = d_fw_err;
     w.bytes = d_bytes;
-    HC(hipMemsetAsync(w.n_big, 0, 4, st));
+    HC(hipMemsetAsync(w.n_big, 0, 4, s));
 #ifdef RS_FWCLK
     w.clk = A.get<unsigned long long>(phase == 1 ? "fw.clk1" : "fw.clk2", 32 + 8 * 64);
-    HC(hipMemsetAsync(w.clk, 0, 8 * (32 + 8 * 64), st));
+    HC(hipMemsetAsync(w.clk, 0, 8 * (32 + 8 * 64), s));
 #endif
     a.xlist = w.big;
     a.n_xlist = w.n_big;
-    HC(hipEventRecord(e0, st));
-    fh_split = split < n;
-    if (fh_split) {
-      w.n = split;
-      launch_capped(st, k_frames_wave<0>, split, kFwBlocks, w);
-      launch(st, k_nl_fill, n, a);
-      HC(hipEventRecord(E->ev_fh[0], st));
-      between();
-      HC(hipMemsetAsync(w.n_big, 0, 4, st));
-      HC(hipEventRecord(E->ev_fh[1], st));
-      w.x0 = split;
-      w.n = n;
-      launch_capped(st, k_frames_wave<0>, n - split, kFwBlocks, w);
-    } else {
-      launch_capped(st, k_frames_wave<0>, n, kFwBlocks, w);
-    }
-    launch(st, k_nl_fill, n, a);
-    HC(hipEventRecord(e1, st));
+    HC(hipEventRecord(e0, s));
+    launch_capped(s, k_frames_wave<0>, n, kFwBlocks, w);
+    launch(s, k_nl_fill, n, a);
+    HC(hipEventRecord(e1, s));
     if (g_prof_env) {
       unsigned nb = 0;
-      HC(hipMemcpyAsync(&nb, w.n_big, 4, hipMemcpyDeviceToHost, st));
-      HC(hipStreamSynchronize(st));
+      HC(hipMemcpyAsync(&nb, w.n_big, 4, hipMemcpyDeviceToHost, s));
+      HC(hipStreamSynchronize(s));
       fprintf(stderr, "[rs-prof] nl phase %d: %u rows over a wave batch\n", phase, nb);
       if (w.clk) {
         unsigned long long c[32 + 8 * 64];
@@ -670,40 +673,126 @@
   void nl_ms(hipEvent_t e0, hipEvent_t e1) {
     float ms = 0;
     HC(hipEventSynchronize(e1));
-    if (fh_split) {
-      float m2 = 0;
-      HC(hipEventElapsedTime(&ms, e0, E->ev_fh[0]));
-      HC(hipEventElapsedTime(&m2, E->ev_fh[1], e1));
-      ms += m2;
-      fh_split = false;
+    HC(hipEventElapsedTime(&ms, e0, e1));
+    E->stats.apply_kernel_ms += ms;
+  }
+  void frames_pass(uint64_t x0, uint64_t n, hipStream_t s, int slot, const char *what) {
+    if (!n) return;
+    if (n_pass >= kMaxPass) throw RsError(RS_E_INTERNAL, "frames passes: more than the engine has events for");
+    const int p = n_pass++;
+    pass_slot[p] = slot;
+    nl_phase(2, nl_lids + x0, n, E->ev_pass[p][0], E->ev_pass[p][1], s, x0, p);
+    if (slot >= 0) E->nlst.nl_pass_start_ms[slot] = pass_host_ms;
+    snap_list(nl_lids + x0, n, x0, s, p, what);
+  }
+  void frames_pass_ms() {
+    for (; n_timed < n_pass; ++n_timed) {
+      hipEvent_t *ev = E->ev_pass[n_timed];
+      float ms = 0, t = 0;
+      HC(hipEventSynchronize(ev[1]));
+      HC(hipEventElapsedTime(&ms, ev[0], ev[1]));
+      HC(hipEventElapsedTime(&t, E->ev_t0, ev[0]));
+      E->stats.apply_kernel_ms += ms;
+      if (pass_slot[n_timed] >= 0) E->nlst.nl_pass_dev_ms[pass_slot[n_timed]] = t;
+    }
+  }
+  std::vector<uint64_t> slice_rows(uint64_t K) const {
+    std::vector<uint64_t> r(K + 1, n_nl);
+    r[0] = 0;
+    const rs_input *in = E->hin;
+    if (K < 2 || !in || !in->nl_a.ptr || !in->nl_b.ptr || !in->nl_c.ptr) return r;
+    auto cum = [&](uint64_t row) { return in->nl_a.ptr[row] + in->nl_b.ptr[row] + in->nl_c.ptr[row]; };
+    const uint64_t tot = cum(n_nl);
+    for (uint64_t i = 1; i < K; ++i) {
+      const uint64_t want = (uint64_t)((unsigned __int128)tot * i / K);
+      uint64_t lo = 0, hi = n_nl;
+      while (lo < hi) {
+        const uint64_t m = lo + (hi - lo) / 2;
+        if (cum(m) < want) lo = m + 1; else hi = m;
+      }
+      r[i] = std::max(r[i - 1], lo);
+    }
+    return r;
+  }
+  void level_lists(hipStream_t s, uint64_t K, uint64_t *cut) {
+    nl_lvl = A.get<uint8_t>("nl.lvl", n_nl);
+    launch(s, k_nl_levels, n_nl, fr, (const uint8_t *)hmark, nl_in[0], nl_in[1], nl_in[2], n_nl, nl_lvl, (uint64_t *)cap3);
+    const U3 t = excl_scan_u3(E, cap3, sc3, n_nl, "lv", nullptr, nullptr, nullptr, s);
+    if (t.a + t.b + t.c != n_nl) throw RsError(RS_E_INTERNAL, "frames levels: the lists do not hold every row");
+    lvl_n[0] = t.a; lvl_n[1] = t.b; lvl_n[2] = t.c;
+    launch(s, k_level_lists, n_nl, (const uint8_t *)nl_lvl, (const uint64_t *)sc3, t.a, t.a + t.b, n_nl, nl_lids);
+    cut[0] = 0;
+    for (uint64_t i = 1; i <= K; ++i) cut[i] = t.a;
+    if (K > 1) {
+      const std::vector<uint64_t> r = slice_rows(K);
+      uint64_t *h = (uint64_t *)pin_get(E, kPinRead, kPinRb);
+      for (uint64_t i = 1; i < K; ++i)
+        if (r[i] < n_nl) HC(hipMemcpyAsync(h + i - 1, &sc3[r[i]].a, 8, hipMemcpyDeviceToHost, s));
+      HC(hipStreamSynchronize(s));
+      for (uint64_t i = 1; i < K; ++i) cut[i] = r[i] < n_nl ? std::min<uint64_t>(h[i - 1], t.a) : t.a;
+      for (uint64_t i = 1; i < K; ++i) cut[i] = std::max(cut[i], cut[i - 1]);
+    }
+    for (int l = 0; l < 3; ++l) E->nlst.nl_level_rows[l] = lvl_n[l];
+    if (g_prof_env)
+      fprintf(stderr, "[rs-prof] levels: rows %llu / %llu / %llu, %llu slice(s) at %.2f ms\n", (unsigned long long)t.a,
+              (unsigned long long)t.b, (unsigned long long)t.c, (unsigned long long)K, now_ms() - T0);
+  }
+  void head_overlap(const uint32_t *ids, uint64_t n_head, uint64_t n_t1, const ElimArgs &ea) {
+    nl_listed = E->stream_out && !(E->comm && E->comm->world > 1);
+    const bool lv3 = nl_listed && env_u64("RS_NL_LEVELS", 1, 0, 1) != 0 &&
+                     n_nl >= env_u64("RS_NL_LEVELS_MIN", 1ull << 20, 0, UINT64_MAX);
+    const uint64_t K = lv3 ? env_u64("RS_NL_SLICES", 2, 1, kMaxSlices) : 1;
+    const hipStream_t s0 = lv3 ? E->ste : st;
+    if (nl_split && nl_listed) {
+      HC(hipStreamSynchronize(E->stc));
+      n_pass = n_timed = 0;
+      E->snap_on = false;
+      HC(hipMemsetAsync(so_early, 0, n_nl, s0));
+    }
+    hmark = A.get<uint8_t>("nl.hmark", E->S);
+    nl_lids = A.get<uint32_t>("nl.lids", n_nl);
+    HC(hipMemsetAsync(hmark, 0, E->S, s0));
+    auto mark = [&](const uint32_t *cl, uint64_t n, uint8_t v) {
+      for (uint64_t o = 0; o < n; o += 32768) {
+        hipLaunchKernelGGL(k_mark_head_keys, dim3(16, (unsigned)std::min<uint64_t>(n - o, 32768)), dim3(256), 0, s0, ea.rows,
+                           (const uint32_t *)ea.perm, (const uint64_t *)ea.cl_off, cl + o, hmark, v);
+        HC(hipGetLastError());
+      }
+    };
+    mark(ids, n_head, 2);
+    if (lv3) mark(ids + n_head, n_t1, 1);
+    fr.h_off = ea.h_off; fr.h_len = ea.h_len; fr.pk = ea.pk; fr.pv = ea.pv;
+    nl_split = true;
+    if (!nl_listed) {
+      nl_late = A.get<uint64_t>("nl.late", n_nl);
+      nl_lpos = A.get<uint64_t>("nl.lpos", n_nl);
+      nl_phase(1, nullptr, n_nl, E->ev[kEvNl0], E->ev[kEvNl1]);
+      snap_take(nl_late);
+      return;
+    }
+    stage_nl();
+    if (lv3) HC(hipStreamWaitEvent(E->ste, E->ev_nlc, 0));
+    uint64_t cut[kMaxSlices + 1];
+    level_lists(s0, K, cut);
+    E->nlst.nl_levels = lv3 ? 3 : 2;
+    E->nlst.nl_slices = K;
+    if (lv3) {
+      for (uint64_t i = 0; i < K; ++i)
+        frames_pass(cut[i], cut[i + 1] - cut[i], E->ste, i == 0 ? 0 : (i == K - 1 ? 1 : -1), "level 0");
+      HC(hipEventRecord(E->ev_l0, E->ste));
+      frames_pass(lvl_n[0], lvl_n[1], st, 2, "level 1");
+      HC(hipStreamWaitEvent(st, E->ev_l0, 0));
     } else {
-      HC(hipEventElapsedTime(&ms, e0, e1));
-    }
-    E->stats.apply_kernel_ms += ms;
-  }
-  void head_overlap(const uint32_t *ids, uint64_t n_head, const ElimArgs &ea) {
-    hmark = A.get<uint8_t>("nl.hmark", E->S);
-    nl_late = A.get<uint64_t>("nl.late", n_nl);
-    nl_lpos = A.get<uint64_t>("nl.lpos", n_nl);
-    nl_lids = A.get<uint32_t>("nl.lids", n_nl);
-    HC(hipMemsetAsync(hmark, 0, E->S, st));
-    hipLaunchKernelGGL(k_mark_head_keys, dim3(16, (unsigned)n_head), dim3(256), 0, st, ea.rows, (const uint32_t *)ea.perm,
-                       (const uint64_t *)ea.cl_off, ids, hmark);
-    HC(hipGetLastError());
-    fr.h_off = ea.h_off; fr.h_len = ea.h_len; fr.pk = ea.pk; fr.pv = ea.pv;
-    const bool halves = E->stream_out && !(E->comm && E->comm->world > 1) &&
-                        n_nl >= env_u64("RS_HALVES_MIN", 1ull << 20, 0, UINT64_MAX) && !env_flag("RS_NO_HALVES");
-    const double frac = env_f64("RS_HALF_FRAC", 0.5, 0.0, 1.0);
-    const uint64_t h = halves ? std::max<uint64_t>(1, std::min<uint64_t>(n_nl - 1, (uint64_t)(n_nl * frac))) : n_nl;
-    nl_phase(1, nullptr, n_nl, E->ev[kEvNl0], E->ev[kEvNl1], h, [&] { snap_take(nl_late, h); });
-    if (!halves) snap_take(nl_late, n_nl);
-    else snap_take_h2(h);
-    nl_split = true;
+      frames_pass(0, lvl_n[0], st, 0, "levels 0-1");
+    }
+    n_late = lvl_n[2];
   }
 
   void linear_round1() {
     P = get_pool(E, 1 << 20);
-    const HeadOverlap overlap = [this](const uint32_t *ids, uint64_t n_head, const ElimArgs &ea) { head_overlap(ids, n_head, ea); };
+    const HeadOverlap overlap = [this](const uint32_t *ids, uint64_t n_head, uint64_t n_t1, const ElimArgs &ea) {
+      head_overlap(ids, n_head, n_t1, ea);
+    };
     const std::function<void()> values = [this] { linear_values(); };
     if (apply_linear) {
       uint8_t *relevant = nullptr;
@@ -735,15 +824,23 @@
     fr.pk = P.pk;
     fr.pv = P.pv;
     if (n_nl) {
-      if (nl_split) nl_ms(E->ev[kEvNl0], E->ev[kEvNl1]);
       if (!nl_split) {
         nl_phase(0, nullptr, n_nl, E->ev[kEvFill0], E->ev[kEvFill1]);
-        snap_take(nullptr, n_nl);
+        snap_take(nullptr);
         nl_ms(E->ev[kEvFill0], E->ev[kEvFill1]);
-      } else if (n_late) {
-        nl_phase(2, nl_lids, n_late, E->ev[kEvFill0], E->ev[kEvFill1]);
-        snap_take2();
-        nl_ms(E->ev[kEvFill0], E->ev[kEvFill1]);
+      } else if (nl_listed) {
+        frames_pass(lvl_n[0] + lvl_n[1], n_late, st, 3, "level 2");
+        frames_pass_ms();
+        if (E->nlst.nl_slices == 1) {
+          E->nlst.nl_pass_start_ms[1] = E->nlst.nl_pass_start_ms[0];
+          E->nlst.nl_pass_dev_ms[1] = E->nlst.nl_pass_dev_ms[0];
+        }
+      } else {
+        nl_ms(E->ev[kEvNl0], E->ev[kEvNl1]);
+        if (n_late) {
+          nl_phase(2, nl_lids, n_late, E->ev[kEvFill0], E->ev[kEvFill1]);
+          nl_ms(E->ev[kEvFill0], E->ev[kEvFill1]);
+        }
       }
     }
     unsigned long long bytes = 0;
@@ -761,6 +858,15 @@
       HC(hipMemcpyAsync(h_wl, d_wl, 8, hipMemcpyDeviceToHost, st));
     }
     HC(hipStreamSynchronize(st));
+    if (g_prof_env && nl_listed && nl_lvl) {
+      unsigned long long *cnt = A.get<unsigned long long>("nl.lcnt", 3), h[3];
+      HC(hipMemsetAsync(cnt, 0, 24, st));
+      launch(st, k_level_entries, n_nl, (const uint8_t *)nl_lvl, (const uint32_t *)stor[0].len, (const uint32_t *)stor[1].len,
+             (const uint32_t *)stor[2].len, n_nl, cnt);
+      HC(hipMemcpyAsync(h, cnt, 24, hipMemcpyDeviceToHost, st));
+      HC(hipStreamSynchronize(st));
+      fprintf(stderr, "[rs-prof] levels: result entries of storage rows %llu / %llu / %llu\n", h[0], h[1], h[2]);
+    }
     if (n_nl) {
       n_wl = h_wl[0];
       if (n_wl > n_nl) throw RsError(RS_E_INTERNAL, "non-linear split: row counts out of range");
@@ -810,7 +916,7 @@
            U3{E->snap_e[0], E->snap_e[1], E->snap_e[2]}, n_st, so_early, so_eoff, so_dirty);
     HC(hipEventRecord(E->ev_snap0, st));
     HC(hipStreamWaitEvent(E->stc, E->ev_snap0, 0));
-    snap_tail(e3, E->ev_snapq + 3, "round snapshot", "", [&](int q, uint32_t *col, uint64_t *val, uint64_t b) {
+    snap_tail(e3, E->ev_snapq + 3 * kMaxPass, "round snapshot", "", [&](int q, uint32_t *col, uint64_t *val, uint64_t b) {
       E->kg[2].run(E->stc, 24 * n_st + 72 * e3[q], [&] {
         launch(E->stc, k_snap_gather_st, n_st, E->F, cp[q], (const U3 *)elen, (const U3 *)eoff3, b, q, n_st, col, val);
       });
diff --git a/include/rs_simplify.h b/include/rs_simplify.h
--- a/include/rs_simplify.h
+++ b/include/rs_simplify.h
@@ -7,7 +7,7 @@
 extern "C" {
 #endif
 
-#define RS_ABI_VERSION 14
+#define RS_ABI_VERSION 15
 
 enum rs_status {
   RS_OK = 0,
@@ -197,6 +197,14 @@
   uint64_t bytes;
 } rs_json_stats;
 
+typedef struct rs_nl_stats {
+  uint64_t nl_level_rows[3];
+  uint64_t nl_levels;
+  uint64_t nl_slices;
+  double nl_pass_start_ms[4];
+  double nl_pass_dev_ms[4];
+} rs_nl_stats;
+
 typedef struct rs_engine rs_engine;
 
 const char *rs_last_error(void);
@@ -247,6 +255,7 @@
 int rs_write_constraints_json_device(int device, const char *path, const rs_output *out);
 int rs_write_substitution_json_device(int device, const char *path, const rs_output *out);
 int rs_engine_json_stats(rs_engine *eng, rs_json_stats *st);
+int rs_engine_nl_stats(rs_engine *eng, rs_nl_stats *st);
 
 typedef struct rs_witness {
   uint32_t prime_id;
diff --git a/integration/rust/src/lib.rs b/integration/rust/src/lib.rs
--- a/integration/rust/src/lib.rs
+++ b/integration/rust/src/lib.rs
@@ -1,7 +1,7 @@
 #![allow(non_camel_case_types)]
 use std::os::raw::{c_char, c_int, c_void};
 
-pub const RS_ABI_VERSION: c_int = 14;
+pub const RS_ABI_VERSION: c_int = 15;
 pub const RS_COMM_ID_BYTES: usize = 128;
 
 pub const RS_OK: c_int = 0;
@@ -222,6 +222,15 @@
 }
 
 #[repr(C)]
+pub struct rs_nl_stats {
+    pub nl_level_rows: [u64; 3],
+    pub nl_levels: u64,
+    pub nl_slices: u64,
+    pub nl_pass_start_ms: [f64; 4],
+    pub nl_pass_dev_ms: [f64; 4],
+}
+
+#[repr(C)]
 pub struct rs_witness {
     pub prime_id: u32,
     pub prime: [u64; 4],
@@ -321,6 +330,7 @@
     pub fn rs_write_constraints_json_device(device: c_int, path: *const c_char, out: *const rs_output) -> c_int;
     pub fn rs_write_substitution_json_device(device: c_int, path: *const c_char, out: *const rs_output) -> c_int;
     pub fn rs_engine_json_stats(eng: *mut rs_engine, st: *mut rs_json_stats) -> c_int;
+    pub fn rs_engine_nl_stats(eng: *mut rs_engine, st: *mut rs_nl_stats) -> c_int;
     pub fn rs_read_wtns(path: *const c_char, w: *mut *mut rs_witness) -> c_int;
     pub fn rs_witness_free(w: *mut rs_witness);
     pub fn rs_write_wtns(path: *const c_char, w: *const rs_witness, out: *const rs_output) -> c_int;
```
